# shenzebang/PDE-inverse-problem

Measured on NVIDIA B200. Metric: particle-steps/s, higher is better.
Workload: dtype bf16 GEMM operands split hi+lo (MLP weights and x; GMM centres, x and softmax weights in the integrator), f32 accumulate / epilogue / state

## Files before the change

pde_inverse_problem_b200/csrc/residual_tensor.cu:

```cuda
#include "mlp_thread.cuh"
#include "residual_common.cuh"
#include "umma.cuh"

namespace pdeip {

int mlp_residual_accumulate_fp32(int set_kind, const ResidualArgs& a, int hidden, cudaStream_t st);

namespace tc {

using namespace umma;

constexpr int H = 32;
constexpr int OP = 48;

constexpr uint32_t C_DW2 = 0, C_DW1 = 48, C_DW0 = 80, C_SLOT0 = 112, SLOT_COLS = 200;
constexpr uint32_t C_S1P1 = 0, C_S1P2 = 16;
constexpr uint32_t C_R = 32;
constexpr uint32_t C_Z0 = C_R + 0, C_Z10 = C_R + 32;
constexpr uint32_t C_Z1 = C_R + 64, C_Z11 = C_R + 96, C_Z21 = C_R + 0;
constexpr uint32_t C_U = C_R + 0, C_U1 = C_R + 48, C_U2 = C_R + 96;
constexpr uint32_t C_S0P = 176;
constexpr uint32_t C_AA2 = C_R + 0, C_AB12 = C_R + 32, C_PZ2 = C_R + 128;
constexpr uint32_t C_AA1 = C_R + 64, C_AB11 = C_R + 96, C_PZ1 = C_R + 0;
constexpr uint32_t C_G = C_R + 16;
constexpr uint32_t C_ZG0 = C_R + 64, C_ZG1 = C_R + 96, C_UG = C_R + 48;
constexpr uint32_t C_AB2 = C_R + 16, C_AA2R = C_R + 96;
constexpr uint32_t C_AB1 = C_R + 48, C_AA1R = C_R + 96;

constexpr uint32_t C_AOP = C_SLOT0 + SLOT_COLS;
constexpr uint32_t C_AOPX = C_AOP + 48;

constexpr int ZC_ZA2 = 0, ZC_ZA1 = 6, ZC_ZA0 = 10, ZC_TA = 14, ZC_TB = 20;
constexpr int AC_T = 0, AC_A1 = 4, AC_C = 8;

template <int DP, int NS>
struct Cfg {
  static constexpr int XC = DP / 8;
  static constexpr int NX = 4 * XC;
  static constexpr int KX = 2 * DP;
  static constexpr int KV = DP < 16 ? 16 : DP;
  static constexpr int XC_HI = 0, XC_LO = XC, XC_V = 2 * XC, XC_G = 3 * XC;
  static constexpr uint32_t RG_X = NX * 128, RG_A = 12 * 128, RG_Z = 24 * 128;
  static constexpr uint32_t SZ_X = 16 * RG_X, SZ_A = 16 * RG_A, SZ_Z = 16 * RG_Z;
  static constexpr uint32_t O_X = 0, O_A1 = O_X + SZ_X, O_A2 = O_A1 + SZ_A, O_Z = O_A2 + SZ_A, SLOT = O_Z + SZ_Z;
#ifndef PDEIP_TC_PIPE_X
#define PDEIP_TC_PIPE_X 1
#endif
#ifndef PDEIP_TC_STAGE
#define PDEIP_TC_STAGE 0
#endif
  static constexpr bool PIPE_X = PDEIP_TC_PIPE_X && NS == 1 && !PDEIP_TC_STAGE;
  static constexpr uint32_t O_X2 = NS * SLOT;
  static constexpr uint32_t RG_T0X = KX / 8 * 128, SZ_T0X = 4 * RG_T0X;
  static constexpr uint32_t RG_T0V = KV / 8 * 128, SZ_T0V = 4 * RG_T0V;
  static constexpr uint32_t RG_T1 = 512, SZ_T1 = 4 * RG_T1, RG_T2 = 512, SZ_T2 = 6 * RG_T2;
  static constexpr uint32_t O_T0XH = NS * SLOT + (PIPE_X ? SZ_X : 0u), O_T0XL = O_T0XH + SZ_T0X, O_T0VH = O_T0XL + SZ_T0X,
                            O_T0VL = O_T0VH + SZ_T0V, O_T1H = O_T0VL + SZ_T0V, O_T1L = O_T1H + SZ_T1,
                            O_T2H = O_T1L + SZ_T1, O_T2L = O_T2H + SZ_T2,
                            O_TGH = O_T2L + SZ_T2, O_TGL = O_TGH + (NS == 1 ? SZ_T1 : 0u),
                            O_BIAS = O_TGL + (NS == 1 ? SZ_T1 : 0u);
  static constexpr uint32_t TP_BYTES = NS == 2 ? 2048 : 4096;
#ifndef PDEIP_TC_STAGE
#define PDEIP_TC_STAGE 0
#endif
  static constexpr uint32_t STAGE_BYTES = (PDEIP_TC_STAGE && NS == 1) ? 128u * 3u * DP * 4u : 0u;
  static constexpr uint32_t O_TRUE = O_BIAS + 512, O_MISC = O_TRUE + TP_BYTES, O_STAGE = O_MISC + 128,
                            TOTAL = O_STAGE + STAGE_BYTES;
  static_assert(TOTAL <= 227u * 1024u && O_STAGE % 128 == 0 && O_X2 % 1024 == 0, "shared-memory budget");
};

#ifndef PDEIP_TC_G_CHAIN_EARLY
#define PDEIP_TC_G_CHAIN_EARLY 1
#endif
#ifndef PDEIP_TC_NLO_FWD
#define PDEIP_TC_NLO_FWD 1
#endif
#ifndef PDEIP_TC_NLO_BWD
#define PDEIP_TC_NLO_BWD 1
#endif
#ifndef PDEIP_TC_LO_FWD
#define PDEIP_TC_LO_FWD true
#endif
constexpr int kEpiThreads = 256;
constexpr int kThreads = kEpiThreads + 32;
constexpr int kLaunchThreads = 384;
#ifndef PDEIP_TC_REGS1_EPI
#define PDEIP_TC_REGS1_EPI 232
#define PDEIP_TC_REGS1_MMA 40
#endif
#ifndef PDEIP_TC_REGS2_EPI
#define PDEIP_TC_REGS2_EPI 208
#define PDEIP_TC_REGS2_MMA 88
#endif
template <int NS>
struct Regs {
  static constexpr int kEpi = NS == 2 ? PDEIP_TC_REGS2_EPI : PDEIP_TC_REGS1_EPI;
  static constexpr int kMma = NS == 2 ? PDEIP_TC_REGS2_MMA : PDEIP_TC_REGS1_MMA;
  static_assert(2 * (kEpi - 168) <= 168 - kMma && kEpi % 8 == 0 && kMma % 8 == 0 && kMma >= 24 && kEpi <= 256,
                "setmaxnreg budgets: an impossible request never returns (the kernel hangs)");
};

template <int V>
struct IC {
  static constexpr int value = V;
};

#ifdef PDEIP_TC_TRACE
constexpr int kTraceTiles = 64;
#define TC_TRACE(k) do { if (trace_on) atomicAdd(reinterpret_cast<unsigned long long*>(trace) + (ph * 2 + s) * 8 + (k), (unsigned long long)clock64()); } while (0)
#define TC_FINE(k) do { if (trace_on && ph == 4) atomicAdd(reinterpret_cast<unsigned long long*>(trace) + 240 + s * 8 + (k), (unsigned long long)clock64()); } while (0)
#define TC_TRACE_DECL_MMA                                                     \
  long long* trace = reinterpret_cast<long long*>(status) + 512;              \
  const bool trace_on = blockIdx.x == 0 && base >= tile_begin + (int64_t)16 * tile_stride && base < tile_begin + (int64_t)(16 + kTraceTiles) * tile_stride
#else
#define TC_TRACE(k) do { } while (0)
#define TC_FINE(k) do { } while (0)
#define TC_TRACE_DECL_MMA do { } while (0)
#endif

#ifdef PDEIP_TC_PROBE
#define TC_PROBE(id, unit0, arr, n)                                                              \
  do {                                                                                           \
    if (probe_on) {                                                                              \
      for (int _i = 0; _i < (n); ++_i) probe[((id) * 128 + row) * 48 + (unit0) + _i] = (arr)[_i]; \
    }                                                                                            \
  } while (0)
#else
#define TC_PROBE(id, unit0, arr, n) do { } while (0)
#endif

template <bool PROXY_FENCE = true>
__device__ __forceinline__ void epi_arrive(int slot) {
  if constexpr (PROXY_FENCE) fence_async_smem();
  fence_before_sync();
  asm volatile("bar.arrive %0, %1;" ::"r"(1 + slot), "n"(kThreads) : "memory");
}
__device__ __forceinline__ void mma_wait_operands(int slot) {
  asm volatile("bar.sync %0, %1;" ::"r"(1 + slot), "n"(kThreads) : "memory");
  fence_after_sync();
}

struct Desc {
  uint32_t lo, hi;
};
__device__ __forceinline__ Desc mk_desc(uint32_t saddr, uint32_t lbo_bytes, uint32_t sbo_bytes) {
  Desc d;
  d.lo = ((saddr >> 4) & 0x3FFFu) | (((lbo_bytes >> 4) & 0x3FFFu) << 16);
  d.hi = ((sbo_bytes >> 4) & 0x3FFFu) | (1u << 14);
  return d;
}
__device__ __forceinline__ Desc mk_desc16(uint32_t base16, uint32_t off_bytes, uint32_t lbo_bytes, uint32_t sbo_bytes) {
  Desc d;
  d.lo = base16 + ((off_bytes >> 4) | (((lbo_bytes >> 4) & 0x3FFFu) << 16));
  d.hi = ((sbo_bytes >> 4) & 0x3FFFu) | (1u << 14);
  return d;
}
__device__ __forceinline__ uint32_t opaque(uint32_t v) {
  uint32_t r;
  asm volatile("mov.u32 %0, %1;" : "=r"(r) : "r"(v));
  return r;
}
__device__ __forceinline__ void mma(uint32_t d_tmem, Desc a, uint32_t a_adv, Desc b, uint32_t b_adv, uint32_t idesc,
                                    uint32_t accumulate) {
  asm volatile(
      "{\n\t"
      ".reg .pred p;\n\t"
      ".reg .b64 da, db;\n\t"
      "mov.b64 da, {%1, %2};\n\t"
      "mov.b64 db, {%3, %4};\n\t"
      "setp.ne.b32 p, %6, 0;\n\t"
      "tcgen05.mma.cta_group::1.kind::f16 [%0], da, db, %5, p;\n\t"
      "}\n" ::"r"(d_tmem),
      "r"(a.lo + (a_adv >> 4)), "r"(a.hi), "r"(b.lo + (b_adv >> 4)), "r"(b.hi), "r"(idesc), "r"(accumulate)
      : "memory");
}

__device__ __forceinline__ void mma_ts(uint32_t d_tmem, uint32_t a_tmem, Desc b, uint32_t b_adv, uint32_t idesc,
                                       uint32_t accumulate) {
  asm volatile(
      "{\n\t"
      ".reg .pred p;\n\t"
      ".reg .b64 db;\n\t"
      "mov.b64 db, {%2, %3};\n\t"
      "setp.ne.b32 p, %5, 0;\n\t"
      "tcgen05.mma.cta_group::1.kind::f16 [%0], [%1], db, %4, p;\n\t"
      "}\n" ::"r"(d_tmem),
      "r"(a_tmem), "r"(b.lo + (b_adv >> 4)), "r"(b.hi), "r"(idesc), "r"(accumulate)
      : "memory");
}
template <int K, int N, int NG, bool LO = true, int NLO = NG>
__device__ __forceinline__ void mm_fwd_ts(const uint32_t (&d)[NG], const uint32_t (&a_col)[NG], Desc w_hi, Desc w_lo) {
  constexpr uint32_t idesc = make_idesc(N, 0, 0);
#pragma unroll
  for (int k = 0; k < K; k += 16)
#pragma unroll
    for (int g = 0; g < NG; ++g) mma_ts(d[g], a_col[g] + (k >> 1), w_hi, k * 16, idesc, k > 0 ? 1u : 0u);
  if constexpr (LO) {
#pragma unroll
    for (int k = 0; k < K; k += 16)
#pragma unroll
      for (int g = 0; g < NLO; ++g) mma_ts(d[g], a_col[g] + (k >> 1), w_lo, k * 16, idesc, 1u);
  }
}
template <int K, int N, int NG, bool LO = true, int NLO = NG>
__device__ __forceinline__ void mm_bwd_ts(const uint32_t (&d)[NG], const uint32_t (&a_col)[NG], Desc w_hi_m, Desc w_lo_m,
                                          uint32_t w_rg) {
  constexpr uint32_t idesc = make_idesc(N, 0, 1);
#pragma unroll
  for (int k = 0; k < K; k += 16)
#pragma unroll
    for (int g = 0; g < NG; ++g) mma_ts(d[g], a_col[g] + (k >> 1), w_hi_m, (k >> 3) * w_rg, idesc, k > 0 ? 1u : 0u);
  if constexpr (LO) {
#pragma unroll
    for (int k = 0; k < K; k += 16)
#pragma unroll
      for (int g = 0; g < NLO; ++g) mma_ts(d[g], a_col[g] + (k >> 1), w_lo_m, (k >> 3) * w_rg, idesc, 1u);
  }
}

template <int K, int N, int NG, bool LO = true, int NLO = NG>
__device__ __forceinline__ void mm_fwd(const uint32_t (&d)[NG], Desc a, const uint32_t (&a_off)[NG], Desc w_hi, Desc w_lo) {
  constexpr uint32_t idesc = make_idesc(N, 0, 0);
#pragma unroll
  for (int k = 0; k < K; k += 16)
#pragma unroll
    for (int g = 0; g < NG; ++g) mma(d[g], a, a_off[g] + k * 16, w_hi, k * 16, idesc, k > 0 ? 1u : 0u);
  if constexpr (LO) {
#pragma unroll
    for (int k = 0; k < K; k += 16)
#pragma unroll
      for (int g = 0; g < NLO; ++g) mma(d[g], a, a_off[g] + k * 16, w_lo, k * 16, idesc, 1u);
  }
}
template <int K, int N, int NG, bool LO = true, int NLO = NG>
__device__ __forceinline__ void mm_bwd(const uint32_t (&d)[NG], Desc a, const uint32_t (&a_off)[NG], Desc w_hi_m,
                                       Desc w_lo_m, uint32_t w_rg) {
  constexpr uint32_t idesc = make_idesc(N, 0, 1);
#pragma unroll
  for (int k = 0; k < K; k += 16)
#pragma unroll
    for (int g = 0; g < NG; ++g) mma(d[g], a, a_off[g] + k * 16, w_hi_m, (k >> 3) * w_rg, idesc, k > 0 ? 1u : 0u);
  if constexpr (LO) {
#pragma unroll
    for (int k = 0; k < K; k += 16)
#pragma unroll
      for (int g = 0; g < NLO; ++g) mma(d[g], a, a_off[g] + k * 16, w_lo_m, (k >> 3) * w_rg, idesc, 1u);
  }
}
template <int N>
__device__ __forceinline__ void mm_outer(uint32_t d, Desc a_m, uint32_t a_off, uint32_t a_rg, Desc b_m, uint32_t b_off,
                                         uint32_t b_rg, uint32_t accumulate) {
  constexpr uint32_t idesc = (make_idesc(N, 1, 1) & ~(0x1Fu << 24)) | ((uint32_t)(64 >> 4) << 24);
#pragma unroll
  for (int k = 0; k < 128; k += 16)
    mma(d, a_m, a_off + (k >> 3) * a_rg, b_m, b_off + (k >> 3) * b_rg, idesc, k > 0 ? 1u : accumulate);
}

__device__ __forceinline__ float tanh_fast(float x) {
  float y;
  asm("tanh.approx.f32 %0, %1;" : "=f"(y) : "f"(x));
  return y;
}

__device__ __forceinline__ uint32_t pack2(float a, float b) {
  __nv_bfloat162 p = __floats2bfloat162_rn(a, b);
  return *reinterpret_cast<uint32_t*>(&p);
}
__device__ __forceinline__ float bf_lo(uint32_t w) { return __uint_as_float(w << 16); }
__device__ __forceinline__ float bf_hi(uint32_t w) { return __uint_as_float(w & 0xffff0000u); }
__device__ __forceinline__ void load_chunk(const uint8_t* tile, uint32_t off, float* v) {
  const uint4 q = *reinterpret_cast<const uint4*>(tile + off);
  v[0] = bf_lo(q.x); v[1] = bf_hi(q.x); v[2] = bf_lo(q.y); v[3] = bf_hi(q.y);
  v[4] = bf_lo(q.z); v[5] = bf_hi(q.z); v[6] = bf_lo(q.w); v[7] = bf_hi(q.w);
}
__device__ __forceinline__ void put_chunk(uint8_t* tile, uint32_t off, const float* v) {
  uint4 q;
  q.x = pack2(v[0], v[1]); q.y = pack2(v[2], v[3]); q.z = pack2(v[4], v[5]); q.w = pack2(v[6], v[7]);
  *reinterpret_cast<uint4*>(tile + off) = q;
}
__device__ __forceinline__ void mbar_expect_tx(uint32_t mbar, uint32_t bytes) {
  asm volatile("mbarrier.arrive.expect_tx.shared::cta.b64 _, [%0], %1;" ::"r"(mbar), "r"(bytes) : "memory");
}
__device__ __forceinline__ void bulk_g2s(uint32_t dst_smem, const void* src, uint32_t bytes, uint32_t mbar) {
  asm volatile("cp.async.bulk.shared::cluster.global.mbarrier::complete_tx::bytes [%0], [%1], %2, [%3];" ::"r"(dst_smem),
               "l"(src), "r"(bytes), "r"(mbar)
               : "memory");
}
__device__ __forceinline__ void tm_st4(uint32_t taddr, const uint32_t* r);
template <bool TS>
__device__ __forceinline__ void put_op(uint8_t* tile, uint32_t off, uint32_t taddr, const float* v) {
  uint4 q;
  q.x = pack2(v[0], v[1]); q.y = pack2(v[2], v[3]); q.z = pack2(v[4], v[5]); q.w = pack2(v[6], v[7]);
  *reinterpret_cast<uint4*>(tile + off) = q;
  if constexpr (TS) tm_st4(taddr, reinterpret_cast<const uint32_t*>(&q));
}
__device__ __forceinline__ void tm_ld8(uint32_t taddr, uint32_t* r) {
  asm volatile("tcgen05.ld.sync.aligned.32x32b.x8.b32 {%0,%1,%2,%3,%4,%5,%6,%7}, [%8];"
               : "=r"(r[0]), "=r"(r[1]), "=r"(r[2]), "=r"(r[3]), "=r"(r[4]), "=r"(r[5]), "=r"(r[6]), "=r"(r[7])
               : "r"(taddr)
               : "memory");
}
__device__ __forceinline__ void tm_ld4(uint32_t taddr, uint32_t* r) {
  asm volatile("tcgen05.ld.sync.aligned.32x32b.x4.b32 {%0,%1,%2,%3}, [%4];"
               : "=r"(r[0]), "=r"(r[1]), "=r"(r[2]), "=r"(r[3])
               : "r"(taddr)
               : "memory");
}
__device__ __forceinline__ void tm_ld16(uint32_t taddr, uint32_t* r) {
  asm volatile(
      "tcgen05.ld.sync.aligned.32x32b.x16.b32 {%0,%1,%2,%3,%4,%5,%6,%7,%8,%9,%10,%11,%12,%13,%14,%15}, [%16];"
      : "=r"(r[0]), "=r"(r[1]), "=r"(r[2]), "=r"(r[3]), "=r"(r[4]), "=r"(r[5]), "=r"(r[6]), "=r"(r[7]), "=r"(r[8]),
        "=r"(r[9]), "=r"(r[10]), "=r"(r[11]), "=r"(r[12]), "=r"(r[13]), "=r"(r[14]), "=r"(r[15])
      : "r"(taddr)
      : "memory");
}
__device__ __forceinline__ void tm_wait_ld() { asm volatile("tcgen05.wait::ld.sync.aligned;" ::: "memory"); }
__device__ __forceinline__ void tm_wait_st() { asm volatile("tcgen05.wait::st.sync.aligned;" ::: "memory"); }
__device__ __forceinline__ void tm_st8(uint32_t taddr, const uint32_t* r) {
  asm volatile("tcgen05.st.sync.aligned.32x32b.x8.b32 [%0], {%1,%2,%3,%4,%5,%6,%7,%8};" ::"r"(taddr), "r"(r[0]),
               "r"(r[1]), "r"(r[2]), "r"(r[3]), "r"(r[4]), "r"(r[5]), "r"(r[6]), "r"(r[7])
               : "memory");
}
__device__ __forceinline__ void tm_st4(uint32_t taddr, const uint32_t* r) {
  asm volatile("tcgen05.st.sync.aligned.32x32b.x4.b32 [%0], {%1,%2,%3,%4};" ::"r"(taddr), "r"(r[0]), "r"(r[1]),
               "r"(r[2]), "r"(r[3])
               : "memory");
}
template <int NU>
__device__ __forceinline__ void tm_ldf(uint32_t taddr, float* v) {
  uint32_t* r = reinterpret_cast<uint32_t*>(v);
  tm_ld16(taddr, r);
  if constexpr (NU == 24) tm_ld8(taddr + 16, r + 16);
}
template <int NU>
__device__ __forceinline__ void tm_ldp(uint32_t taddr, uint32_t* r) {
  tm_ld8(taddr, r);
  if constexpr (NU == 24) tm_ld4(taddr + 8, r + 8);
}
template <int NU>
__device__ __forceinline__ void tm_park(uint32_t taddr, const float* v) {
  uint32_t r[NU / 2];
#pragma unroll
  for (int i = 0; i < NU / 2; ++i) r[i] = pack2(v[2 * i], v[2 * i + 1]);
  if constexpr (NU == 8) {
    tm_st4(taddr, r);
  } else {
    tm_st8(taddr, r);
    if constexpr (NU == 24) tm_st4(taddr + 8, r + 8);
  }
  tm_wait_st();
}

template <int DP>
__device__ __noinline__ void true_grad_chunk(const ResidualArgs& a, const float* __restrict__ tp, int64_t p, int dimw,
                                             int cg, float* gt) {
  const int d = a.d;
  float x[DP];
#pragma unroll
  for (int u = 0; u < DP; ++u)
    x[u] = (p >= 0 && u < d) ? __ldg(a.points + elem_index(a.layout, p, u, a.n_points, dimw)) : 0.f;
  if (a.tg.kind == PDEIP_DRIFT_LINEAR) {
#pragma unroll
    for (int e = 0; e < 8; ++e) {
      const int u = cg * 8 + e;
      float acc = 0.f;
      if (u < d) {
#pragma unroll
        for (int k = 0; k < DP; ++k)
          if (k < d) acc = fmaf(tp[u * d + k], x[k], acc);
      }
      gt[e] = acc;
    }
  } else {
    float m = -INFINITY;
    for (int k = 0; k < a.tg.n_gaussian; ++k) {
      float s2 = 0.f;
#pragma unroll
      for (int u = 0; u < DP; ++u)
        if (u < d) {
          const float r = x[u] - tp[k * d + u];
          s2 = fmaf(r, r, s2);
        }
      m = fmaxf(m, -0.5f * a.tg.inv_sigma2 * s2);
    }
    float se = 0.f, wm[8];
#pragma unroll
    for (int e = 0; e < 8; ++e) wm[e] = 0.f;
    for (int k = 0; k < a.tg.n_gaussian; ++k) {
      float s2 = 0.f;
#pragma unroll
      for (int u = 0; u < DP; ++u)
        if (u < d) {
          const float r = x[u] - tp[k * d + u];
          s2 = fmaf(r, r, s2);
        }
      const float ek = __expf(-0.5f * a.tg.inv_sigma2 * s2 - m);
      se += ek;
#pragma unroll
      for (int e = 0; e < 8; ++e)
        if (cg * 8 + e < d) wm[e] = fmaf(ek, tp[k * d + cg * 8 + e], wm[e]);
    }
    const float inv = 1.f / se;
#pragma unroll
    for (int e = 0; e < 8; ++e) gt[e] = (cg * 8 + e < d) ? (x[cg * 8 + e] - wm[e] * inv) * a.tg.inv_sigma2 : 0.f;
  }
}
__device__ __forceinline__ float unp(const uint32_t* r, int i) { return (i & 1) ? bf_hi(r[i >> 1]) : bf_lo(r[i >> 1]); }

#ifndef PDEIP_TC_PACKED
#define PDEIP_TC_PACKED 1
#endif
__device__ __forceinline__ float2 pr(const float* v, int i) { return make_float2(v[2 * i], v[2 * i + 1]); }
__device__ __forceinline__ void st2(float* v, int i, float2 x) { v[2 * i] = x.x; v[2 * i + 1] = x.y; }
__device__ __forceinline__ float2 unp2(const uint32_t* r, int i) { return make_float2(bf_lo(r[i]), bf_hi(r[i])); }
__device__ __forceinline__ float2 bc2(float x) { return make_float2(x, x); }

constexpr int kModeKfp0T = 0, kModeBnd = 1, kModeFp0T = 2;
template <int DP, int NS, int MODE>
__global__ void __launch_bounds__(kLaunchThreads, 1) mlp_residual_tc_kernel(const ResidualArgs a, int* status) {
  constexpr bool BND = MODE == kModeBnd, FPM = MODE == kModeFp0T;
#ifndef PDEIP_TC_TS
#define PDEIP_TC_TS 1
#endif
  constexpr bool kTS = PDEIP_TC_TS && NS == 1;
#ifndef PDEIP_TC_GRAM
#define PDEIP_TC_GRAM 1
#endif
  constexpr bool kGram = PDEIP_TC_GRAM && NS == 1;
#ifndef PDEIP_TC_TWO_STAGE
#define PDEIP_TC_TWO_STAGE 1
#endif
  constexpr bool kTwoStage = PDEIP_TC_TWO_STAGE && kTS;
  constexpr bool kPipeX = Cfg<DP, NS>::PIPE_X;
  constexpr bool kPipeFlow = kPipeX;
  using S = Cfg<DP, NS>;
  extern __shared__ __align__(1024) uint8_t sm[];
  const int tid = threadIdx.x, warp = tid >> 5, lane = tid & 31;
  const bool is_mma_warp = warp == kEpiThreads / 32;
  const int q = warp & 3;
  const int half = (warp >> 2) & 1;
  const int row = q * 32 + lane;
  const int d = a.d;
  const MlpShape<H> sh{d, 2};
  const int P = sh.num_params();
  float* bias_s = reinterpret_cast<float*>(sm + S::O_BIAS);
  float* tp = reinterpret_cast<float*>(sm + S::O_TRUE);
  uint64_t* mbar_p = reinterpret_cast<uint64_t*>(sm + S::O_MISC);
  uint32_t* tmem_p = reinterpret_cast<uint32_t*>(sm + S::O_MISC + 64);

  const uint32_t fpd = FPM ? (uint32_t)a.fp_dirs : 1u;
  const int64_t n_tiles_all = (a.n_points + 127) / 128 * fpd;
  const int64_t per_cta = ((n_tiles_all + gridDim.x - 1) / gridDim.x + NS - 1) / NS * NS;
  const int64_t tile_begin = (int64_t)blockIdx.x * per_cta;
  if (tile_begin >= n_tiles_all) return;
  const int64_t n_tiles = tile_begin + per_cta < n_tiles_all ? tile_begin + per_cta : n_tiles_all;

  if (warp == 0) {
    tmem_alloc(smem_u32(tmem_p), 512);
    tmem_relinquish();
  }
  if (tid == 0) {
    for (int s = 0; s < NS; ++s) mbar_init(smem_u32(mbar_p + s), 1);
    mbar_init(smem_u32(mbar_p + 4), 1);
    fence_mbar_init();
  }
  for (uint32_t o = tid * 16; o < S::O_BIAS; o += kLaunchThreads * 16) *reinterpret_cast<uint4*>(sm + o) = make_uint4(0, 0, 0, 0);
  if constexpr (S::PIPE_X)
    for (uint32_t o = tid * 16; o < S::SZ_X; o += kLaunchThreads * 16) *reinterpret_cast<uint4*>(sm + S::O_X2 + o) = make_uint4(0, 0, 0, 0);
  __syncthreads();
  {
    const float* W0 = a.params + sh.w_off(0);
    const float* W1 = a.params + sh.w_off(1);
    const float* W2 = a.params + sh.w_off(2);
    auto put = [&](uint32_t o_hi, uint32_t o_lo, uint32_t rg, int r, int c, float w) {
      const __nv_bfloat16 hi = __float2bfloat16_rn(w);
      const __nv_bfloat16 lo = __float2bfloat16_rn(w - __bfloat162float(hi));
      const uint32_t off = chunk_off(r, c >> 3, rg) + (uint32_t)(c & 7) * 2u;
      *reinterpret_cast<__nv_bfloat16*>(sm + o_hi + off) = hi;
      *reinterpret_cast<__nv_bfloat16*>(sm + o_lo + off) = lo;
    };
    for (int idx = tid; idx < 32 * S::KX; idx += kLaunchThreads) {
      const int r = idx / S::KX, c = idx % S::KX, ci = c % DP;
      put(S::O_T0XH, S::O_T0XL, S::RG_T0X, r, c, ci < d ? W0[ci * H + r] : 0.f);
    }
    for (int idx = tid; idx < 32 * S::KV; idx += kLaunchThreads) {
      const int r = idx / S::KV, c = idx % S::KV;
      put(S::O_T0VH, S::O_T0VL, S::RG_T0V, r, c, c < d ? W0[c * H + r] : 0.f);
    }
    for (int idx = tid; idx < 32 * 32; idx += kLaunchThreads) {
      const int r = idx / 32, c = idx % 32;
      put(S::O_T1H, S::O_T1L, S::RG_T1, r, c, W1[c * H + r]);
    }
    for (int idx = tid; idx < OP * 32; idx += kLaunchThreads) {
      const int r = idx / 32, c = idx % 32;
      put(S::O_T2H, S::O_T2L, S::RG_T2, r, c, r < kOut ? W2[c * kOut + r] : 0.f);
    }
    if constexpr (kGram) {
      const float sc = 0.125f / (float)fpd;
      for (int idx = tid; idx < 32 * 32; idx += kLaunchThreads) {
        const int r = idx / 32, c = idx % 32;
        float acc = 0.f;
        for (int k = 0; k < d; ++k) acc = fmaf(W0[k * H + r], W0[k * H + c], acc);
        put(S::O_TGH, S::O_TGL, S::RG_T1, r, c, sc * acc);
      }
    }
    for (int j = tid; j < 32; j += kLaunchThreads) {
      bias_s[j] = a.params[sh.b_off(0) + j];
      bias_s[32 + j] = a.params[sh.b_off(1) + j];
    }
    for (int j = tid; j < OP; j += kLaunchThreads) bias_s[64 + j] = j < kOut ? a.params[sh.b_off(2) + j] : 0.f;
    int ntg = 0;
    if (a.tg.kind == PDEIP_DRIFT_LINEAR) ntg = d * d;
    else if (a.tg.kind == PDEIP_DRIFT_GMM) ntg = a.tg.n_gaussian * d;
    for (int i = tid; i < ntg; i += kLaunchThreads) tp[i] = a.tg.params[i];
  }
  fence_async_smem();
  fence_before_sync();
  __syncthreads();
  fence_after_sync();

  const uint32_t TB = *tmem_p;
  const int64_t tile_stride = NS;

  if (warp >= kEpiThreads / 32) {
    asm volatile("setmaxnreg.dec.sync.aligned.u32 %0;" ::"n"(Regs<NS>::kMma));
  }
  if (is_mma_warp) {
    const uint32_t sm16 = smem_u32(sm) >> 4;
    constexpr uint32_t CH = 128;
    uint32_t dw_started = 0;
    constexpr bool kCChainsEarly = PDEIP_TC_G_CHAIN_EARLY && NS == 2;
    constexpr int kNloFwd = BND ? 2 : PDEIP_TC_NLO_FWD;
    constexpr int kNloBwd = BND ? 2 : PDEIP_TC_NLO_BWD;
    uint32_t xb = 0;
    uint32_t tsb = 0;
#pragma unroll 1
    for (int64_t base = tile_begin; base < n_tiles; base += tile_stride) {
#pragma unroll 1
      for (int ph = (kPipeFlow && base != tile_begin) ? 1 : 0; ph < 12; ++ph) {
        if (kGram && ph == 6) continue;
#pragma unroll 1
        for (int s = 0; s < NS; ++s) {
          const uint32_t w16 = opaque(sm16), b16 = opaque(sm16 + (uint32_t)s * (S::SLOT >> 4));
          const uint32_t x16 = kPipeX ? opaque(sm16 + (xb ? (S::O_X2 >> 4) : 0u)) : b16;
          const uint32_t x16n = kPipeX ? opaque(sm16 + (xb ? 0u : (S::O_X2 >> 4))) : b16;
          const uint32_t TBo = opaque(TB);
          const uint32_t TS = TBo + C_SLOT0 + (uint32_t)s * SLOT_COLS;
          const uint32_t mb = smem_u32(mbar_p + s);
          const uint32_t AOP = TBo + C_AOP;
          const Desc T0XHK = mk_desc16(w16, S::O_T0XH, 128, S::RG_T0X), T0XLK = mk_desc16(w16, S::O_T0XL, 128, S::RG_T0X);
          const Desc T0VHK = mk_desc16(w16, S::O_T0VH, 128, S::RG_T0V), T0VLK = mk_desc16(w16, S::O_T0VL, 128, S::RG_T0V);
          const Desc T1HK = mk_desc16(w16, S::O_T1H, 128, S::RG_T1), T1LK = mk_desc16(w16, S::O_T1L, 128, S::RG_T1);
          const Desc T2HK = mk_desc16(w16, S::O_T2H, 128, S::RG_T2), T2LK = mk_desc16(w16, S::O_T2L, 128, S::RG_T2);
          const Desc TGHK = mk_desc16(w16, S::O_TGH, 128, S::RG_T1), TGLK = mk_desc16(w16, S::O_TGL, 128, S::RG_T1);
          const Desc T0VHM = mk_desc16(w16, S::O_T0VH, S::RG_T0V, 128), T0VLM = mk_desc16(w16, S::O_T0VL, S::RG_T0V, 128);
          const Desc T1HM = mk_desc16(w16, S::O_T1H, S::RG_T1, 128), T1LM = mk_desc16(w16, S::O_T1L, S::RG_T1, 128);
          const Desc T2HM = mk_desc16(w16, S::O_T2H, S::RG_T2, 128), T2LM = mk_desc16(w16, S::O_T2L, S::RG_T2, 128);
          const Desc XK = mk_desc16(x16, S::O_X, 128, S::RG_X), A1K = mk_desc16(b16, S::O_A1, 128, S::RG_A),
                     A2K = mk_desc16(b16, S::O_A2, 128, S::RG_A), ZK = mk_desc16(b16, S::O_Z, 128, S::RG_Z);
          const Desc XM = mk_desc16(x16, S::O_X, S::RG_X, 128), ZM = mk_desc16(b16, S::O_Z, S::RG_Z, 128);
          const uint32_t AOPX = kPipeX ? TBo + C_AOPX : AOP;
          auto issue_p0 = [&](const Desc xk) {
            if constexpr (kTS) {
              mm_fwd_ts<S::KX, 32, 1>({TS + C_Z0}, {AOPX}, T0XHK, T0XLK);
              mm_fwd_ts<S::KV, 32, 1, (PDEIP_TC_NLO_FWD >= 2 || BND)>({TS + C_Z10}, {AOPX + S::KX / 2}, T0VHK, T0VLK);
            } else {
              mm_fwd<S::KX, 32, 1>({TS + C_Z0}, xk, {S::XC_HI * CH}, T0XHK, T0XLK);
              mm_fwd<S::KV, 32, 1, (PDEIP_TC_NLO_FWD >= 2 || BND)>({TS + C_Z10}, xk, {S::XC_V * CH}, T0VHK, T0VLK);
            }
          };
          TC_TRACE_DECL_MMA;
          mma_wait_operands(s);
          if (elect_one()) {
            TC_TRACE(4);
            switch (ph) {
              case 0: {
                issue_p0(XK);
                commit(mb);
              } break;
              case 1: {
                if constexpr (kTS) mm_fwd_ts<32, 32, 3, PDEIP_TC_LO_FWD, kNloFwd>({TS + C_Z1, TS + C_Z11, TS + C_Z21}, {AOP + 4 * AC_T, AOP + 4 * AC_A1, AOP + 4 * AC_C}, T1HK, T1LK);
                else mm_fwd<32, 32, 3, PDEIP_TC_LO_FWD, kNloFwd>({TS + C_Z1, TS + C_Z11, TS + C_Z21}, A1K, {AC_T * CH, AC_A1 * CH, AC_C * CH}, T1HK, T1LK);
                commit(mb);
              } break;
              case 2: {
                if constexpr (kTS) mm_fwd_ts<32, OP, 3, PDEIP_TC_LO_FWD, kNloFwd>({TS + C_U, TS + C_U1, TS + C_U2}, {AOP + 4 * AC_T, AOP + 4 * AC_A1, AOP + 4 * AC_C}, T2HK, T2LK);
                else mm_fwd<32, OP, 3, PDEIP_TC_LO_FWD, kNloFwd>({TS + C_U, TS + C_U1, TS + C_U2}, A2K, {AC_T * CH, AC_A1 * CH, AC_C * CH}, T2HK, T2LK);
                commit(mb);
              } break;
              case 3: {
                if constexpr (kTS) mm_bwd_ts<OP, 32, 2, true, kNloBwd>({TS + C_AA2, TS + C_AB12}, {AOP, AOP + 24}, T2HM, T2LM, S::RG_T2);
                else mm_bwd<OP, 32, 2, true, kNloBwd>({TS + C_AA2, TS + C_AB12}, ZK, {ZC_ZA2 * CH, ZC_TA * CH}, T2HM, T2LM, S::RG_T2);
                commit(mb);
              } break;
              case 4: {
                if constexpr (kTS) mm_bwd_ts<32, 32, 2, true, kNloBwd>({TS + C_AA1, TS + C_AB11}, {AOP, AOP + 16}, T1HM, T1LM, S::RG_T1);
                else mm_bwd<32, 32, 2, true, kNloBwd>({TS + C_AA1, TS + C_AB11}, ZK, {ZC_ZA1 * CH, ZC_TB * CH}, T1HM, T1LM, S::RG_T1);
                commit(mb);
              } break;
              case 5: {
                if constexpr (kTS) mm_bwd_ts<32, S::KV, 1>({TS + C_G}, {AOP}, T0VHM, T0VLM, S::RG_T0V);
                else mm_bwd<32, S::KV, 1>({TS + C_G}, ZK, {ZC_ZA0 * CH}, T0VHM, T0VLM, S::RG_T0V);
                if constexpr (kGram) {
                  if constexpr (kTS) mm_fwd_ts<32, 32, 1, true>({TS + C_ZG0}, {AOP}, TGHK, TGLK);
                  else mm_fwd<32, 32, 1, true>({TS + C_ZG0}, ZK, {ZC_ZA0 * CH}, TGHK, TGLK);
                }
                commit(mb);
              } break;
              case 6: {
                if constexpr (kTS) mm_fwd_ts<S::KV, 32, 1, false>({TS + C_ZG0}, {AOP}, T0VHK, T0VLK);
                else mm_fwd<S::KV, 32, 1, false>({TS + C_ZG0}, XK, {S::XC_G * CH}, T0VHK, T0VLK);
                commit(mb);
#if PDEIP_TC_G_CHAIN_EARLY
                mm_outer<32>(TBo + C_DW0, XM, S::XC_G * CH, S::RG_X, ZM, ZC_ZA0 * CH, S::RG_Z, 1u);
#endif
              } break;
              case 7: {
                if constexpr (kTS) mm_fwd_ts<32, 32, 1, false>({TS + C_ZG1}, {AOP}, T1HK, T1LK);
                else mm_fwd<32, 32, 1, false>({TS + C_ZG1}, A1K, {AC_A1 * CH}, T1HK, T1LK);
                commit(mb);
                if constexpr (kGram && !kTwoStage)
                  mm_outer<32>(TBo + C_DW0, XM, S::XC_G * CH, S::RG_X, ZM, ZC_ZA0 * CH, S::RG_Z, 1u);
                if constexpr (kCChainsEarly) {
                  const Desc A1M = mk_desc16(b16, S::O_A1, S::RG_A, 128);
                  mm_outer<32>(TBo + C_DW1, A1M, AC_C * CH, S::RG_A, ZM, ZC_ZA1 * CH, S::RG_Z, 1u);
                }
              } break;
              case 8: {
                if constexpr (kTS) mm_fwd_ts<32, OP, 1, false>({TS + C_UG}, {AOP}, T2HK, T2LK);
                else mm_fwd<32, OP, 1, false>({TS + C_UG}, A2K, {AC_A1 * CH}, T2HK, T2LK);
                commit(mb);
                if constexpr (kCChainsEarly) {
                  const Desc A2M = mk_desc16(b16, S::O_A2, S::RG_A, 128);
                  mm_outer<OP>(TBo + C_DW2, A2M, AC_C * CH, S::RG_A, ZM, ZC_ZA2 * CH, S::RG_Z, 1u);
                }
              } break;
              case 9: {
                if constexpr (kTS) {
                  mm_bwd_ts<OP, 32, 1, BND, 1>({TS + C_AB2}, {AOP}, T2HM, T2LM, S::RG_T2);
                  mm_bwd<OP, 32, 1, false>({TS + C_AA2R}, ZK, {ZC_ZA2 * CH}, T2HM, T2LM, S::RG_T2);
                } else {
                  mm_bwd<OP, 32, 2, BND, 1>({TS + C_AB2, TS + C_AA2R}, ZK, {ZC_TA * CH, ZC_ZA2 * CH}, T2HM, T2LM, S::RG_T2);
                }
                commit(mb);
              } break;
              case 10: {
                if constexpr (kTS) {
                  mm_bwd_ts<32, 32, 1, BND, 1>({TS + C_AB1}, {AOP}, T1HM, T1LM, S::RG_T1);
                  mm_bwd<32, 32, 1, false>({TS + C_AA1R}, ZK, {ZC_ZA1 * CH}, T1HM, T1LM, S::RG_T1);
                } else {
                  mm_bwd<32, 32, 2, BND, 1>({TS + C_AB1, TS + C_AA1R}, ZK, {ZC_TB * CH, ZC_ZA1 * CH}, T1HM, T1LM, S::RG_T1);
                }
                commit(mb);
              } break;
              default: {
                const bool p0_next = kPipeFlow && base + tile_stride < n_tiles;
                if (p0_next) {
                  issue_p0(mk_desc16(x16n, S::O_X, 128, S::RG_X));
                  commit(mb);
                }
                if constexpr (!kTwoStage) {
                  mm_outer<32>(TBo + C_DW0, XM, S::XC_HI * CH, S::RG_X, ZM, ZC_TA * CH, S::RG_Z, 1u);
#ifdef PDEIP_TC_XLO_DW
                  mm_outer<32>(TBo + C_DW0, XM, S::XC_LO * CH, S::RG_X, ZM, ZC_TA * CH, S::RG_Z, 1u);
#endif
#if !PDEIP_TC_G_CHAIN_EARLY
                  mm_outer<32>(TBo + C_DW0, XM, S::XC_G * CH, S::RG_X, ZM, ZC_ZA0 * CH, S::RG_Z, 1u);
#endif
                  if (!p0_next) commit(mb);
                }
              } break;
            }
            TC_TRACE(6);
          }
          __syncwarp();
        }
        if (ph == 3 || ph == 4 || ph == 5 || ph == 9 || ph == 10 || (kTwoStage && (ph == 7 || ph == 11))) {
#pragma unroll 1
          for (int s = 0; s < NS; ++s) {
            if constexpr (kTwoStage) {
              asm volatile("bar.sync %0, %1;" ::"r"(4 + (int)tsb), "n"(kThreads) : "memory");
              tsb ^= 1u;
              fence_after_sync();
            }
            const uint32_t b16 = opaque(sm16 + (uint32_t)s * (S::SLOT >> 4)), TBo = opaque(TB);
            const uint32_t x16 = kPipeX ? opaque(sm16 + (xb ? (S::O_X2 >> 4) : 0u)) : b16;
            const Desc XM = mk_desc16(x16, S::O_X, S::RG_X, 128), A1M = mk_desc16(b16, S::O_A1, S::RG_A, 128),
                       A2M = mk_desc16(b16, S::O_A2, S::RG_A, 128), ZM = mk_desc16(b16, S::O_Z, S::RG_Z, 128);
            const uint32_t acc_first = (dw_started | (uint32_t)s) ? 1u : 0u;
            if (elect_one()) {
              switch (ph) {
                case 3:
                  mm_outer<OP>(TBo + C_DW2, A2M, AC_A1 * CH, S::RG_A, ZM, ZC_TA * CH, S::RG_Z, acc_first);
                  break;
                case 4:
                  mm_outer<32>(TBo + C_DW1, A1M, AC_A1 * CH, S::RG_A, ZM, ZC_TB * CH, S::RG_Z, acc_first);
                  break;
                case 5:
                  mm_outer<32>(TBo + C_DW0, XM, S::XC_V * CH, S::RG_X, ZM, ZC_TA * CH, S::RG_Z, acc_first);
                  break;
                case 9:
                  mm_outer<OP>(TBo + C_DW2, A2M, AC_T * CH, S::RG_A, ZM, ZC_TA * CH, S::RG_Z, 1u);
                  if constexpr (!kCChainsEarly)
                    mm_outer<OP>(TBo + C_DW2, A2M, AC_C * CH, S::RG_A, ZM, ZC_ZA2 * CH, S::RG_Z, 1u);
                  break;
                case 10:
                  mm_outer<32>(TBo + C_DW1, A1M, AC_T * CH, S::RG_A, ZM, ZC_TB * CH, S::RG_Z, 1u);
                  if constexpr (!kCChainsEarly)
                    mm_outer<32>(TBo + C_DW1, A1M, AC_C * CH, S::RG_A, ZM, ZC_ZA1 * CH, S::RG_Z, 1u);
                  break;
                case 7:
                  if constexpr (kGram) mm_outer<32>(TBo + C_DW0, XM, S::XC_G * CH, S::RG_X, ZM, ZC_ZA0 * CH, S::RG_Z, 1u);
                  break;
                default: {
                  mm_outer<32>(TBo + C_DW0, XM, S::XC_HI * CH, S::RG_X, ZM, ZC_TA * CH, S::RG_Z, 1u);
#ifdef PDEIP_TC_XLO_DW
                  mm_outer<32>(TBo + C_DW0, XM, S::XC_LO * CH, S::RG_X, ZM, ZC_TA * CH, S::RG_Z, 1u);
#endif
#if !PDEIP_TC_G_CHAIN_EARLY
                  mm_outer<32>(TBo + C_DW0, XM, S::XC_G * CH, S::RG_X, ZM, ZC_ZA0 * CH, S::RG_Z, 1u);
#endif
                  if (!(kPipeFlow && base + tile_stride < n_tiles)) commit(smem_u32(mbar_p + s));
                } break;
              }
            }
            __syncwarp();
          }
        }
      }
      dw_started = 1u;
      xb ^= 1u;
    }
  } else if (warp < kEpiThreads / 32) {
    asm volatile("setmaxnreg.inc.sync.aligned.u32 %0;" ::"n"(Regs<NS>::kEpi));
    bool ok = true;
    uint32_t par = 0;
#ifdef PDEIP_TC_PROBE
    float* probe = reinterpret_cast<float*>(status) + 2048;
#endif
    float db0[16], db1[16], db2[24];
#pragma unroll
    for (int i = 0; i < 16; ++i) { db0[i] = 0.f; db1[i] = 0.f; }
#pragma unroll
    for (int i = 0; i < 24; ++i) db2[i] = 0.f;
    float sum_g2 = 0.f, sum_gt2 = 0.f, sum_gd2 = 0.f, sum_d1 = 0.f, sum_d2 = 0.f;
    const float gamma = a.coef, gamma4 = 4.f * a.coef;
    const float cgw = 1.f / (float)fpd;
    const int dimw = (FPM ? d : 2 * d) + (a.tg.kind == PDEIP_DRIFT_IN_POINTS ? d : 0);
    const uint32_t offX = (uint32_t)(row & 7) * 16u + (uint32_t)(row >> 3) * S::RG_X;
    const uint32_t offA = (uint32_t)(row & 7) * 16u + (uint32_t)(row >> 3) * S::RG_A;
    const uint32_t offZ = (uint32_t)(row & 7) * 16u + (uint32_t)(row >> 3) * S::RG_Z;
    const uint32_t LA0 = TB + ((uint32_t)(q * 32) << 16) + C_SLOT0;
    const uint32_t LOP = TB + ((uint32_t)(q * 32) << 16) + C_AOP;
    const int u16 = 16 * half, u24 = 24 * half;
    constexpr int NI = (3 * S::XC + 1) / 2;
    float xin0[NI][8], xin1[NI][8];
    const bool fast_in = !FPM && a.layout == PDEIP_LAYOUT_BLOCK128 && d == DP;
    auto load_into = [&](float (&xin)[NI][8], int64_t t, const int i0 = 0, const int i1 = 64) {
      if (fast_in) {
        const int64_t pp = t * 128 + row;
        const bool inside = t < n_tiles && pp < a.n_points;
        const float* const pb = a.points + (inside ? t * (int64_t)(128 * dimw) + row : (int64_t)0) + half * (8 * 128);
        const bool has_gt = a.tg.kind == PDEIP_DRIFT_IN_POINTS;
#pragma unroll
        for (int i = 0; i < NI; ++i) {
          if (i < i0 || i >= i1) continue;
          if (half + 2 * i >= 3 * S::XC) continue;
          if (half + 2 * i >= 2 * S::XC && !has_gt) continue;
#pragma unroll
          for (int e = 0; e < 8; ++e) xin[i][e] = __ldg(pb + (16 * i + e) * 128);
        }
        return;
      }
      const int64_t cstride = comp_stride(a.layout, a.n_points);
      const uint32_t tq = FPM ? (uint32_t)t / fpd : 0u;
      const int dir = FPM ? (int)((uint32_t)t - tq * fpd) : -1;
      const int64_t pp = (FPM ? (int64_t)tq : t) * 128 + row;
      const int64_t pc = (t < n_tiles && pp < a.n_points) ? pp : 0;
      const float* const pbase = a.points + point_base(a.layout, pc, dimw);
#pragma unroll
      for (int i = 0; i < NI; ++i) {
        if (i < i0 || i >= i1) continue;
        const int j = half + 2 * i;
        const int band = (j / S::XC) < 3 ? (j / S::XC) : 0, cg = j % S::XC;
        const int bandc = (band < 2 || a.tg.kind == PDEIP_DRIFT_IN_POINTS) ? band : 0;
        const int bandm = FPM ? (bandc == 2 ? 1 : 0) : bandc;
#pragma unroll
        for (int e = 0; e < 8; ++e) {
          const int u = cg * 8 + e;
          const int uc = u < d ? u : 0;
          const float val = __ldg(pbase + (bandm * d + uc) * cstride);
          xin[i][e] = (FPM && band == 1) ? (u == dir ? 1.f : 0.f) : val;
        }
      }
    };
    constexpr bool kStage = PDEIP_TC_STAGE && NS == 1;
    const bool use_stage = kStage && a.layout == PDEIP_LAYOUT_BLOCK128 && (reinterpret_cast<uintptr_t>(a.points) & 15u) == 0;
    const float* const stage = reinterpret_cast<const float*>(sm + S::O_STAGE) + row;
    const uint32_t stage_mbar = smem_u32(mbar_p + 4);
    uint32_t spar = 0;
    auto stage_issue = [&](int64_t t) {
      if (t >= n_tiles) return;
      const int64_t pt = FPM ? (int64_t)((uint32_t)t / fpd) : t;
      const uint32_t bytes = 512u * (uint32_t)dimw;
      mbar_expect_tx(stage_mbar, bytes);
      bulk_g2s(smem_u32(sm + S::O_STAGE), a.points + pt * 128 * dimw, bytes, stage_mbar);
    };
    if (use_stage && tid == 0) stage_issue(tile_begin);
    auto load_inputs = [&](int s, int64_t t, const int i0 = 0, const int i1 = 64) {
      if (NS == 2 && s == 1) load_into(xin1, t, i0, i1);
      else load_into(xin0, t, i0, i1);
    };
#ifndef PDEIP_TC_L2_PREFETCH
#define PDEIP_TC_L2_PREFETCH 1
#endif
    auto prefetch_inputs = [&](int64_t t) {
      if (FPM || t >= n_tiles || (t + 1) * 128 > a.n_points) return;
      if (a.layout == PDEIP_LAYOUT_SOA) {
        if ((a.n_points & 3) == 0 && half == 0 && row < dimw)
          asm volatile("cp.async.bulk.prefetch.L2.global [%0], %1;" ::"l"(a.points + (int64_t)row * a.n_points + t * 128),
                       "r"(512u)
                       : "memory");
      } else if (half == 0 && row == 0) {
        asm volatile("cp.async.bulk.prefetch.L2.global [%0], %1;" ::"l"(a.points + t * 128 * dimw),
                     "r"((uint32_t)(512 * dimw))
                     : "memory");
      }
    };
#if !PDEIP_TC_L2_PREFETCH
    load_inputs(0, tile_begin);
    if constexpr (NS == 2) load_inputs(1, tile_begin + 1);
#endif

    bool first = true;
    int64_t base = tile_begin;
    uint32_t xb = 0;
    uint32_t tsb = 0;
    const uint32_t LOPX = kPipeX ? TB + ((uint32_t)(q * 32) << 16) + C_AOPX : LOP;
    auto emit_x = [&](const float (&xin)[NI][8], const bool valid_t, uint8_t* const Xd) {
#pragma unroll
      for (int i = 0; i < NI; ++i) {
        const int j = half + 2 * i;
        const int band = j / S::XC, cg = j % S::XC;
        if (band == 0) {
          float hi[8], lo[8];
#pragma unroll
          for (int e = 0; e < 8; ++e) {
            const float xv = (valid_t && cg * 8 + e < d) ? xin[i][e] : 0.f;
            hi[e] = __bfloat162float(__float2bfloat16_rn(xv));
            lo[e] = xv - hi[e];
          }
          put_op<kTS>(Xd, (S::XC_HI + cg) * 128, LOPX + 4 * cg, hi);
          put_op<kTS>(Xd, (S::XC_LO + cg) * 128, LOPX + 4 * (S::XC + cg), lo);
        } else if (band == 1) {
          float vv[8];
#pragma unroll
          for (int e = 0; e < 8; ++e) vv[e] = (valid_t && cg * 8 + e < d) ? xin[i][e] : 0.f;
          put_op<kTS>(Xd, (S::XC_V + cg) * 128, LOPX + S::KX / 2 + 4 * cg, vv);
        }
      }
    };

    auto phase = [&](auto PHc, const int s) {
      constexpr int ph = decltype(PHc)::value;
      uint8_t* const X = sm + (kPipeX ? (xb ? S::O_X2 : 0u) : (uint32_t)s * S::SLOT) + S::O_X + offX;
      uint8_t* const A1 = sm + (uint32_t)s * S::SLOT + S::O_A1 + offA;
      uint8_t* const A2 = sm + (uint32_t)s * S::SLOT + S::O_A2 + offA;
      uint8_t* const Z = sm + (uint32_t)s * S::SLOT + S::O_Z + offZ;
      const uint32_t LA = LA0 + (uint32_t)s * SLOT_COLS;
      const int64_t tile = base + s;
      const int64_t p = (FPM ? (int64_t)((uint32_t)tile / fpd) : tile) * 128 + row;
      const bool valid = tile < n_tiles && p < a.n_points;
      const float mk = valid ? 1.f : 0.f;
#ifdef PDEIP_TC_PROBE
      const bool probe_on = blockIdx.x == 0 && tile == 0;
#endif
#ifdef PDEIP_TC_TRACE
      long long* trace = reinterpret_cast<long long*>(status) + 512;
      const bool trace_on = blockIdx.x == 0 && tid == 0 && base >= tile_begin + (int64_t)16 * tile_stride &&
                            base < tile_begin + (int64_t)(16 + kTraceTiles) * tile_stride;
#endif
      auto wait_gemm = [&]() {
        TC_TRACE(0);
        if (!(ph == 0 && first)) {
          if (ok && !mbar_wait(smem_u32(mbar_p + s), (par >> s) & 1u)) {
            ok = false;
            atomicExch(status, 1);
          }
          par ^= 1u << s;
          TC_TRACE(3);
          fence_after_sync();
        }
        TC_TRACE(1);
      };
      constexpr bool kEarlyLoads = true;
#if PDEIP_TC_L2_PREFETCH
      if constexpr (ph == 0) {
        if (!use_stage) load_inputs(s, tile);
      }
#endif
      if constexpr (kStage && ph == 0) {
        if (use_stage) {
          if (ok && !mbar_wait(stage_mbar, spar)) {
            ok = false;
            atomicExch(status, 1);
          }
          spar ^= 1u;
          const int dir = FPM ? (int)((uint32_t)tile % fpd) : -1;
#pragma unroll
          for (int i = 0; i < NI; ++i) {
            const int j = half + 2 * i;
            const int band = (j / S::XC) < 3 ? (j / S::XC) : 0, cg = j % S::XC;
            if (band < 2) {
#pragma unroll
              for (int e = 0; e < 8; ++e) {
                const int u = cg * 8 + e;
                const float val = stage[(band * d + (u < d ? u : 0)) * 128];
                xin0[i][e] = (FPM && band == 1) ? (u == dir ? 1.f : 0.f) : val;
              }
            }
          }
        }
      }
      if constexpr (ph <= 3 || ph == 6 || !kEarlyLoads) wait_gemm();
      if constexpr (ph == 0) {
        if (NS == 2 && s == 1) emit_x(xin1, valid, X);
        else emit_x(xin0, valid, X);
      } else if constexpr (ph == 1 || ph == 2) {
        constexpr bool l1 = ph == 1;
        uint8_t* const At = l1 ? A1 : A2;
        float z0[16], z1[16], z2[16];
        tm_ldf<16>(LA + (l1 ? C_Z0 : C_Z1) + u16, z0);
        tm_ldf<16>(LA + (l1 ? C_Z10 : C_Z11) + u16, z1);
        if constexpr (!l1) tm_ldf<16>(LA + C_Z21 + u16, z2);
        float bb[16];
#pragma unroll
        for (int i = 0; i < 4; ++i)
          *reinterpret_cast<float4*>(bb + 4 * i) = *reinterpret_cast<const float4*>(bias_s + (l1 ? 0 : 32) + u16 + 4 * i);
        tm_wait_ld();
        float t[16], s1[16], q1[16], q2[16];
#if PDEIP_TC_PACKED
#pragma unroll
        for (int i = 0; i < 8; ++i) {
          const float2 zb = __fadd2_rn(pr(z0, i), pr(bb, i));
          const float2 t2 = make_float2(tanh_fast(zb.x), tanh_fast(zb.y));
          const float2 s2 = __ffma2_rn(__fmul2_rn(t2, bc2(-1.f)), t2, bc2(1.f));
          const float2 z12 = pr(z1, i);
          const float2 q = __fmul2_rn(s2, z12);
          float2 r = __fmul2_rn(__fmul2_rn(t2, q), z12);
          if constexpr (!l1) r = __ffma2_rn(s2, pr(z2, i), r);
          st2(t, i, t2); st2(s1, i, s2); st2(q1, i, q); st2(q2, i, r);
        }
#else
#pragma unroll
        for (int i = 0; i < 16; ++i) {
          t[i] = tanh_fast(z0[i] + bb[i]);
          s1[i] = fmaf(-t[i], t[i], 1.f);
          q1[i] = s1[i] * z1[i];
          const float w = t[i] * q1[i];
          q2[i] = l1 ? w * z1[i] : fmaf(s1[i], z2[i], w * z1[i]);
        }
#endif
#pragma unroll
        for (int c = 0; c < 2; ++c) {
          put_op<kTS>(At, (AC_T + 2 * half + c) * 128, LOP + 4 * (AC_T + 2 * half + c), t + 8 * c);
          put_op<kTS>(At, (AC_A1 + 2 * half + c) * 128, LOP + 4 * (AC_A1 + 2 * half + c), q1 + 8 * c);
          put_op<kTS>(At, (AC_C + 2 * half + c) * 128, LOP + 4 * (AC_C + 2 * half + c), q2 + 8 * c);
        }
        tm_park<16>(LA + (l1 ? C_S1P1 : C_S1P2) + 8 * half, s1);
        TC_PROBE(l1 ? 0 : 3, u16, t, 16);
        TC_PROBE(l1 ? 1 : 4, u16, q1, 16);
        TC_PROBE(l1 ? 2 : 5, u16, q2, 16);
      } else if constexpr (ph == 3) {
        float u[24], u1[24], u2[24];
        tm_ldf<24>(LA + C_U + u24, u);
        tm_ldf<24>(LA + C_U1 + u24, u1);
        tm_ldf<24>(LA + C_U2 + u24, u2);
        float bb[24];
#pragma unroll
        for (int i = 0; i < 6; ++i)
          *reinterpret_cast<float4*>(bb + 4 * i) = *reinterpret_cast<const float4*>(bias_s + 64 + u24 + 4 * i);
        tm_wait_ld();
        const float k8 = BND ? 0.f : 8.f * mk, kg = (BND ? 2.f * a.coef : gamma4) * mk;
        float d1 = 0.f, d2a = 0.f, d2b = 0.f;
        float za[24], sv[24], sp[24];
#if PDEIP_TC_PACKED
        {
          float2 e1 = bc2(0.f), e2a = bc2(0.f), e2b = bc2(0.f);
          const float2 k82 = bc2(k8), nk82 = bc2(-k8), kg2 = bc2(kg);
#pragma unroll
          for (int i = 0; i < 12; ++i) {
            const float2 uu = __fadd2_rn(pr(u, i), pr(bb, i));
            const float2 v1 = pr(u1, i), v2 = pr(u2, i);
            e1 = __ffma2_rn(uu, v1, e1);
            e2a = __ffma2_rn(v1, v1, e2a);
            e2b = __ffma2_rn(uu, v2, e2b);
            st2(za, i, __fmul2_rn(k82, uu));
            st2(sv, i, __ffma2_rn(nk82, v1, __fmul2_rn(kg2, uu)));
            st2(sp, i, __ffma2_rn(k82, v2, __fmul2_rn(kg2, v1)));
          }
          d1 = e1.x + e1.y; d2a = e2a.x + e2a.y; d2b = e2b.x + e2b.y;
        }
#else
#pragma unroll
        for (int i = 0; i < 24; ++i) {
          const float uu = u[i] + bb[i];
          d1 = fmaf(uu, u1[i], d1);
          d2a = fmaf(u1[i], u1[i], d2a);
          d2b = fmaf(uu, u2[i], d2b);
          za[i] = k8 * uu;
          sv[i] = fmaf(-k8, u1[i], kg * uu);
          sp[i] = fmaf(k8, u2[i], kg * u1[i]);
        }
#endif
#pragma unroll
        for (int c = 0; c < 3; ++c) {
          put_op<kTS>(Z, (ZC_ZA2 + 3 * half + c) * 128, LOP + 4 * (3 * half + c), za + 8 * c);
          put_op<kTS>(Z, (ZC_TA + 3 * half + c) * 128, LOP + 24 + 4 * (3 * half + c), sv + 8 * c);
        }
        tm_park<24>(LA + C_S0P + 12 * half, sp);
        sum_d1 = fmaf(2.f * mk, d1, sum_d1);
        sum_d2 = fmaf(mk, 2.f * d2a - 4.f * d2b, sum_d2);
        TC_PROBE(6, u24, za, 24);
        TC_PROBE(7, u24, sv, 24);
        TC_PROBE(8, u24, sp, 24);
      } else if constexpr (ph == 4 || ph == 5) {
        if constexpr (kPipeFlow && ph == 4) prefetch_inputs(tile + tile_stride);
        constexpr bool l2 = ph == 4;
        const uint8_t* At = l2 ? A2 : A1;
        float aa[16], ab1[16], t[16], a1[16];
        uint32_t s1p[8];
        tm_ldp<16>(LA + (l2 ? C_S1P2 : C_S1P1) + 8 * half, s1p);
#pragma unroll
        for (int c = 0; c < 2; ++c) {
          load_chunk(At, (AC_T + 2 * half + c) * 128, t + 8 * c);
          load_chunk(At, (AC_A1 + 2 * half + c) * 128, a1 + 8 * c);
        }
        tm_wait_ld();
        if constexpr (kEarlyLoads) wait_gemm();
        tm_ldf<16>(LA + (l2 ? C_AA2 : C_AA1) + u16, aa);
        tm_ldf<16>(LA + (l2 ? C_AB12 : C_AB11) + u16, ab1);
        tm_wait_ld();
        TC_FINE(0);
        float za[16], zb[16], pz[16];
#if PDEIP_TC_PACKED
#pragma unroll
        for (int i = 0; i < 8; ++i) {
          const float2 s2 = unp2(s1p, i), aa2 = pr(aa, i), a12 = pr(a1, i), ab2 = pr(ab1, i);
          const float2 tt = __fmul2_rn(pr(t, i), bc2(2.f));
          const float2 qq = __fmul2_rn(aa2, a12);
          st2(za, i, __fmul2_rn(aa2, s2));
          st2(zb, i, __ffma2_rn(tt, qq, __fmul2_rn(s2, ab2)));
          st2(pz, i, __fmul2_rn(a12, __ffma2_rn(__fmul2_rn(tt, bc2(-1.f)), ab2, qq)));
        }
#else
#pragma unroll
        for (int i = 0; i < 16; ++i) {
          const float s1 = unp(s1p, i);
          za[i] = aa[i] * s1;
          const float qq = aa[i] * a1[i];
          zb[i] = fmaf(2.f * t[i], qq, s1 * ab1[i]);
          pz[i] = a1[i] * fmaf(-2.f * t[i], ab1[i], qq);
        }
#endif
#pragma unroll
        for (int c = 0; c < 2; ++c) {
          put_op<kTS>(Z, ((l2 ? ZC_ZA1 : ZC_ZA0) + 2 * half + c) * 128, LOP + 4 * (2 * half + c), za + 8 * c);
          put_op<(kTS && l2)>(Z, ((l2 ? ZC_TB : ZC_TA) + 2 * half + c) * 128, LOP + 16 + 4 * (2 * half + c), zb + 8 * c);
        }
        TC_FINE(1);
        tm_park<16>(LA + (l2 ? C_PZ2 : C_PZ1) + 8 * half, pz);
        TC_FINE(2);
        TC_PROBE(l2 ? 9 : 12, u16, za, 16);
        TC_PROBE(l2 ? 10 : 13, u16, zb, 16);
        TC_PROBE(l2 ? 11 : 14, u16, pz, 16);
      } else if constexpr (ph == 6) {
#pragma unroll
        for (int i = 0; i < NI; ++i) {
          const int j = half + 2 * i;
          const int band = j / S::XC, cg = j % S::XC;
          const bool own_sum = a.tg.kind == PDEIP_DRIFT_IN_POINTS ? band == 2 : band == 0;
          if (j < 3 * S::XC && (band == 0 || own_sum)) {
            float g4[8], gv[8], gt[8];
            tm_ld8(LA + C_G + 8 * cg, reinterpret_cast<uint32_t*>(g4));
            tm_wait_ld();
#pragma unroll
            for (int e = 0; e < 8; ++e) {
              gv[e] = 0.25f * g4[e];
              gt[e] = 0.f;
            }
            if (band == 0) {
              float gh[8];
#pragma unroll
              for (int e = 0; e < 8; ++e) gh[e] = (0.125f * cgw) * g4[e];
              put_op<kTS>(X, (S::XC_G + cg) * 128, LOP + 4 * cg, gh);
              TC_PROBE(15, cg * 8, gv, 8);
            }
            if (own_sum) {
              const float mkc = mk * cgw;
              if (a.tg.kind == PDEIP_DRIFT_IN_POINTS) {
#pragma unroll
                for (int e = 0; e < 8; ++e) {
                  const int u = cg * 8 + e;
                  float val;
                  if (kStage && use_stage) val = stage[((FPM ? d : 2 * d) + (u < d ? u : 0)) * 128];
                  else val = (NS == 2 && s == 1) ? xin1[i][e] : xin0[i][e];
                  gt[e] = (valid && u < d) ? val : 0.f;
                }
              } else if (a.tg.kind == PDEIP_DRIFT_LINEAR || a.tg.kind == PDEIP_DRIFT_GMM) {
                true_grad_chunk<DP>(a, tp, valid ? p : (int64_t)-1, dimw, cg, gt);
              }
#pragma unroll
              for (int e = 0; e < 8; ++e) {
                const float df = gt[e] - gv[e];
                sum_g2 = fmaf(mkc * gv[e], gv[e], sum_g2);
                sum_gt2 = fmaf(mkc * gt[e], gt[e], sum_gt2);
                sum_gd2 = fmaf(mkc * df, df, sum_gd2);
              }
            }
          }
        }
      } else if constexpr (ph == 7 || ph == 8) {
        constexpr bool l1 = ph == 7;
        uint8_t* const At = l1 ? A1 : A2;
        float zg[16], a2[16];
        uint32_t s1p[8];
        tm_ldp<16>(LA + (l1 ? C_S1P1 : C_S1P2) + 8 * half, s1p);
#pragma unroll
        for (int c = 0; c < 2; ++c) load_chunk(At, (AC_C + 2 * half + c) * 128, a2 + 8 * c);
        tm_wait_ld();
        if constexpr (kEarlyLoads && !(kGram && l1)) wait_gemm();
        if constexpr (kStage && l1) {
          if (use_stage && tid == 0) stage_issue(tile + tile_stride);
        }
        tm_ldf<16>(LA + (l1 ? C_ZG0 : C_ZG1) + u16, zg);
        tm_wait_ld();
        float ag[16], cc[16];
#if PDEIP_TC_PACKED
#pragma unroll
        for (int i = 0; i < 8; ++i) {
          const float2 g2 = __fmul2_rn(unp2(s1p, i), pr(zg, i));
          st2(ag, i, g2);
          st2(cc, i, __fadd2_rn(pr(a2, i), g2));
        }
#else
#pragma unroll
        for (int i = 0; i < 16; ++i) {
          ag[i] = unp(s1p, i) * zg[i];
          cc[i] = a2[i] + ag[i];
        }
#endif
#pragma unroll
        for (int c = 0; c < 2; ++c) {
          put_op<kTS>(At, (AC_A1 + 2 * half + c) * 128, LOP + 4 * (2 * half + c), ag + 8 * c);
          put_chunk(At, (AC_C + 2 * half + c) * 128, cc + 8 * c);
        }
        TC_PROBE(l1 ? 16 : 17, u16, cc, 16);
      } else if constexpr (ph == 9) {
        float ug[24], s0[24];
        uint32_t spp[12];
        tm_ldp<24>(LA + C_S0P + 12 * half, spp);
        tm_wait_ld();
        if constexpr (kEarlyLoads) wait_gemm();
        tm_ldf<24>(LA + C_UG + u24, ug);
        tm_wait_ld();
#if PDEIP_TC_PACKED
#pragma unroll
        for (int i = 0; i < 12; ++i) {
          const float2 v = __ffma2_rn(bc2(8.f), pr(ug, i), unp2(spp, i));
          st2(s0, i, v);
          st2(db2, i, __fadd2_rn(pr(db2, i), v));
        }
#else
#pragma unroll
        for (int i = 0; i < 24; ++i) {
          s0[i] = fmaf(8.f, ug[i], unp(spp, i));
          db2[i] += s0[i];
        }
#endif
#pragma unroll
        for (int c = 0; c < 3; ++c) put_op<kTS>(Z, (ZC_TA + 3 * half + c) * 128, LOP + 4 * (3 * half + c), s0 + 8 * c);
        TC_PROBE(18, u24, s0, 24);
      } else {
        constexpr bool l2 = ph == 10;
#if PDEIP_TC_L2_PREFETCH
        if constexpr (l2) {
          if constexpr (kPipeFlow) {
            if (tile + tile_stride < n_tiles) load_inputs(s, tile + tile_stride, 0, 2);
          } else if (!use_stage) {
            prefetch_inputs(tile + tile_stride);
          }
        }
#else
        if constexpr (l2) load_inputs(s, tile + tile_stride);
#endif
        const uint8_t* At = l2 ? A2 : A1;
        float ab[16], aa[16], t[16], cc[16];
        uint32_t s1p[8], pzp[8];
        tm_ldp<16>(LA + (l2 ? C_S1P2 : C_S1P1) + 8 * half, s1p);
        tm_ldp<16>(LA + (l2 ? C_PZ2 : C_PZ1) + 8 * half, pzp);
#pragma unroll
        for (int c = 0; c < 2; ++c) {
          load_chunk(At, (AC_T + 2 * half + c) * 128, t + 8 * c);
          load_chunk(At, (AC_C + 2 * half + c) * 128, cc + 8 * c);
        }
        tm_wait_ld();
        if constexpr (kEarlyLoads) wait_gemm();
        tm_ldf<16>(LA + (l2 ? C_AB2 : C_AB1) + u16, ab);
        tm_ldf<16>(LA + (l2 ? C_AA2R : C_AA1R) + u16, aa);
        tm_wait_ld();
        float zb[16];
#if PDEIP_TC_PACKED
#pragma unroll
        for (int i = 0; i < 8; ++i) {
          const float2 m0 = __ffma2_rn(unp2(s1p, i), pr(ab, i), unp2(pzp, i));
          const float2 ta = __fmul2_rn(__fmul2_rn(pr(t, i), bc2(-2.f)), pr(aa, i));
          const float2 v = __ffma2_rn(ta, pr(cc, i), m0);
          st2(zb, i, v);
          if (l2) st2(db1, i, __fadd2_rn(pr(db1, i), v));
          else st2(db0, i, __fadd2_rn(pr(db0, i), v));
        }
#else
#pragma unroll
        for (int i = 0; i < 16; ++i) {
          const float m0 = fmaf(unp(s1p, i), ab[i], unp(pzp, i));
          zb[i] = fmaf(-2.f * t[i] * aa[i], cc[i], m0);
          if (l2) db1[i] += zb[i];
          else db0[i] += zb[i];
        }
#endif
#pragma unroll
        for (int c = 0; c < 2; ++c)
          put_op<(kTS && l2)>(Z, ((l2 ? ZC_TB : ZC_TA) + 2 * half + c) * 128, LOP + 4 * (2 * half + c), zb + 8 * c);
        TC_PROBE(l2 ? 19 : 20, u16, zb, 16);
      }
      if constexpr (!(kGram && ph == 6)) {
        if constexpr (kTS) tm_wait_st();
        TC_TRACE(7);
        if constexpr (kTwoStage && (ph == 3 || ph == 4 || ph == 5 || ph == 7 || ph == 9 || ph == 10 || ph == 11)) {
          epi_arrive<false>(s);
          fence_async_smem();
          asm volatile("bar.arrive %0, %1;" ::"r"(4 + (int)tsb), "n"(kThreads) : "memory");
          tsb ^= 1u;
        } else {
#ifdef PDEIP_TC_TRACE
        fence_async_smem();
        TC_FINE(3);
        fence_before_sync();
        TC_FINE(4);
        asm volatile("bar.arrive %0, %1;" ::"r"(1 + s), "n"(kThreads) : "memory");
#else
        constexpr bool kNeedProxyFence = !(kTS && (ph == 0 || ph == 1 || ph == 2 || ph == 8));
        epi_arrive<kNeedProxyFence>(s);
#endif
        }
        TC_TRACE(2);
      }
      if constexpr (kPipeFlow && ph == 10) {
        const int64_t tn = tile + tile_stride;
        const int64_t pn = (FPM ? (int64_t)((uint32_t)tn / fpd) : tn) * 128 + row;
        if (tn < n_tiles) {
          load_inputs(s, tn, 2, 64);
          emit_x(xin0, pn < a.n_points, sm + (xb ? 0u : S::O_X2) + S::O_X + offX);
        }
      }
    };
#define PDEIP_TC_PHASE(PH)                       \
  _Pragma("unroll 1") for (int s_ = 0; s_ < NS; ++s_) phase(IC<PH>{}, s_);

#pragma unroll 1
    for (; base < n_tiles; base += tile_stride) {
      if (!kPipeFlow || first) { PDEIP_TC_PHASE(0) }
      PDEIP_TC_PHASE(1) PDEIP_TC_PHASE(2) PDEIP_TC_PHASE(3) PDEIP_TC_PHASE(4) PDEIP_TC_PHASE(5)
      PDEIP_TC_PHASE(6) PDEIP_TC_PHASE(7) PDEIP_TC_PHASE(8) PDEIP_TC_PHASE(9) PDEIP_TC_PHASE(10) PDEIP_TC_PHASE(11)
      first = false;
      xb ^= 1u;
    }
#undef PDEIP_TC_PHASE
#pragma unroll
    for (int s = 0; s < NS; ++s) {
      if (ok && !mbar_wait(smem_u32(mbar_p + s), (par >> s) & 1u)) {
        ok = false;
        atomicExch(status, 1);
      }
    }
    fence_after_sync();
    asm volatile("bar.sync 3, %0;" ::"n"(kEpiThreads) : "memory");

    float* part = a.ws + (int64_t)blockIdx.x * a.pstride;
    float* red = reinterpret_cast<float*>(sm);
    const float wt = a.weight;
    if (ok && q < 2) {
      const uint32_t LQ = TB + ((uint32_t)(q * 32) << 16);
      const int iu = 16 * q + lane;
      float w2[24], w1[16], w0[16];
      tm_ldf<24>(LQ + C_DW2 + u24, w2);
      tm_ldf<16>(LQ + C_DW1 + u16, w1);
      tm_ldf<16>(LQ + C_DW0 + u16, w0);
      tm_wait_ld();
      if (lane < 16) {
#pragma unroll
        for (int i = 0; i < 24; ++i)
          if (u24 + i < kOut) part[sh.w_off(2) + iu * kOut + u24 + i] += wt * w2[i];
#pragma unroll
        for (int i = 0; i < 16; ++i) part[sh.w_off(1) + iu * H + u16 + i] += wt * w1[i];
        if (iu < d) {
#pragma unroll
          for (int i = 0; i < 16; ++i) part[sh.w_off(0) + iu * H + u16 + i] += wt * w0[i];
        }
      }
    }
#pragma unroll
    for (int i = 0; i < 16; ++i) {
      const float r0 = warp_sum(db0[i]), r1 = warp_sum(db1[i]);
      if (lane == 0) {
        red[q * 128 + u16 + i] = r0;
        red[q * 128 + 32 + u16 + i] = r1;
      }
    }
#pragma unroll
    for (int i = 0; i < 24; ++i) {
      const float r2 = warp_sum(db2[i]);
      if (lane == 0) red[q * 128 + 64 + u24 + i] = r2;
    }
    {
      const float sums5[5] = {sum_g2, sum_gt2, sum_gd2, sum_d1, sum_d2};
#pragma unroll
      for (int k = 0; k < 5; ++k) {
        const float sk = warp_sum(sums5[k]);
        if (lane == 0) red[512 + warp * 8 + k] = sk;
      }
    }
    asm volatile("bar.sync 3, %0;" ::"n"(kEpiThreads) : "memory");
    if (ok) {
      if (tid < 112) {
        const float v = (red[tid] + red[128 + tid]) + (red[256 + tid] + red[384 + tid]);
        if (tid < 32) part[sh.b_off(0) + tid] += wt * v;
        else if (tid < 64) part[sh.b_off(1) + tid - 32] += wt * v;
        else if (tid - 64 < kOut) part[sh.b_off(2) + tid - 64] += wt * v;
      }
      if (tid == 128) {
        float t5[5] = {0.f, 0.f, 0.f, 0.f, 0.f};
        for (int w = 0; w < kEpiThreads / 32; ++w)
          for (int k = 0; k < 5; ++k) t5[k] += red[512 + w * 8 + k];
        const float g2 = wt * t5[0], gt2 = wt * t5[1], gd2 = wt * t5[2], D1 = wt * t5[3], D2 = wt * t5[4];
        if constexpr (BND) {
          part[P + PDEIP_SUM_BOUNDARY] += a.coef * D1;
          part[P + PDEIP_SUM_LOSS] += a.coef * D1;
        } else {
          part[P + PDEIP_SUM_G2] += g2;
          part[P + PDEIP_SUM_GTRUE2] += gt2;
          part[P + PDEIP_SUM_GT] += gd2;
          if (!FPM) part[P + PDEIP_SUM_D1] += D1;
          part[P + PDEIP_SUM_D2] += D2;
          part[P + PDEIP_SUM_LOSS] += g2 + gt2 - 2.f * D2 + 2.f * gamma * D1;
        }
      }
    }
  }
  fence_before_sync();
  __syncthreads();
  if (warp == 0) tmem_dealloc(TB, 512);
}

}

int* tensor_status_word() {
  static int* w[64] = {nullptr};
  int dev = 0;
  if (cudaGetDevice(&dev) != cudaSuccess || dev < 0 || dev >= 64) return nullptr;
  if (!w[dev]) {
    const size_t bytes = 8192 + 24 * 128 * 48 * sizeof(float);
    if (cudaMalloc(&w[dev], bytes) != cudaSuccess) return nullptr;
    cudaMemset(w[dev], 0, bytes);
  }
  return w[dev];
}

#ifdef PDEIP_HAVE_TENSOR_PATH
template <int DP, int NS, int MODE>
static int launch_tc(const ResidualArgs& a, int* status, cudaStream_t st) {
  using S = tc::Cfg<DP, NS>;
  auto kern = tc::mlp_residual_tc_kernel<DP, NS, MODE>;
  PDEIP_REQUIRE(true_grad_floats(a.tg, a.d) * sizeof(float) <= S::TP_BYTES, PDEIP_ERR_UNSUPPORTED,
                "tensor path: true-gradient parameters exceed %u bytes", (unsigned)S::TP_BYTES);
  PDEIP_CUDA_OK(cudaFuncSetAttribute(kern, cudaFuncAttributeMaxDynamicSharedMemorySize, (int)S::TOTAL));
  kern<<<residual_grid(), tc::kLaunchThreads, S::TOTAL, st>>>(a, status);
  PDEIP_LAUNCH_OK();
  return PDEIP_OK;
}

int mlp_residual_accumulate_tensor(int set_kind, const ResidualArgs& a, int hidden, cudaStream_t st) {
  if (set_kind != PDEIP_SET_KFP_0T && set_kind != PDEIP_SET_FP_0T && set_kind != PDEIP_SET_KFP_BOUNDARY)
    return mlp_residual_accumulate_fp32(set_kind, a, hidden, st);
  PDEIP_REQUIRE(hidden == 32 && a.layers == 2, PDEIP_ERR_UNSUPPORTED,
                "tensor path is built for hidden_dim == 32, layers == 2 (got %d, %d)", hidden, a.layers);
  PDEIP_REQUIRE(a.d >= 1 && a.d <= 32, PDEIP_ERR_UNSUPPORTED, "tensor path supports 1 <= d <= 32 (got %d)", a.d);
  int* status = tensor_status_word();
  PDEIP_REQUIRE(status != nullptr, PDEIP_ERR_CUDA, "cannot allocate the tensor-path status word");
  ResidualArgs b = a;
  int mode = tc::kModeKfp0T;
  if (set_kind == PDEIP_SET_FP_0T) {
    PDEIP_REQUIRE((a.n_points + 127) / 128 * (int64_t)a.d < ((int64_t)1 << 31), PDEIP_ERR_UNSUPPORTED,
                  "FP tensor path: n_points * d / 128 must stay below 2^31");
    b.fp_dirs = a.d;
    b.coef = 0.f;
    mode = tc::kModeFp0T;
  } else if (set_kind == PDEIP_SET_KFP_BOUNDARY) {
    b.tg.kind = PDEIP_DRIFT_NONE;
    mode = tc::kModeBnd;
  }
#define PDEIP_TC_DISPATCH(DP, NS)                                                     \
  (mode == tc::kModeKfp0T ? launch_tc<DP, NS, tc::kModeKfp0T>(b, status, st)          \
   : mode == tc::kModeBnd ? launch_tc<DP, NS, tc::kModeBnd>(b, status, st)            \
                          : launch_tc<DP, NS, tc::kModeFp0T>(b, status, st))
  if (a.d <= 8) return PDEIP_TC_DISPATCH(8, 2);
  if (a.d <= 16) return PDEIP_TC_DISPATCH(16, 1);
  return PDEIP_TC_DISPATCH(32, 1);
#undef PDEIP_TC_DISPATCH
}
#endif

int tensor_path_status(cudaStream_t st, int* out) {
  int* status = tensor_status_word();
  if (!status) return PDEIP_ERR_CUDA;
  int w[2] = {0, 0};
  if (cudaMemcpyAsync(w, status, 2 * sizeof(int), cudaMemcpyDeviceToHost, st) != cudaSuccess) return PDEIP_ERR_CUDA;
  if (cudaStreamSynchronize(st) != cudaSuccess) return PDEIP_ERR_CUDA;
  *out = (w[0] ? 1 : 0) | (w[1] ? 2 : 0);
  if (*out && cudaMemsetAsync(status, 0, 2 * sizeof(int), st) != cudaSuccess) return PDEIP_ERR_CUDA;
  return PDEIP_OK;
}

}

extern "C" int pdeip_tensor_path_status(void* stream, int* out_status) {
  PDEIP_REQUIRE(out_status != nullptr, PDEIP_ERR_INVALID_ARG, "out_status is NULL");
  return pdeip::tensor_path_status((cudaStream_t)stream, out_status);
}

extern "C" int pdeip_debug_set_status(int word, int value, void* stream) {
  int* status = pdeip::tensor_status_word();
  if (!status || word < 0 || word > 1) return PDEIP_ERR_INVALID_ARG;
  if (cudaMemcpyAsync(status + word, &value, sizeof(int), cudaMemcpyHostToDevice, (cudaStream_t)stream) != cudaSuccess)
    return PDEIP_ERR_CUDA;
  if (cudaStreamSynchronize((cudaStream_t)stream) != cudaSuccess) return PDEIP_ERR_CUDA;
  return PDEIP_OK;
}

extern "C" int pdeip_debug_tensor_trace(long long* out, int n) {
  int* status = pdeip::tensor_status_word();
  if (!status) return PDEIP_ERR_CUDA;
  if (n > 24 * 8 + 48 + 16) return PDEIP_ERR_INVALID_ARG;
  if (cudaDeviceSynchronize() != cudaSuccess) return PDEIP_ERR_CUDA;
  if (cudaMemcpy(out, reinterpret_cast<long long*>(status) + 512, sizeof(long long) * (size_t)n, cudaMemcpyDeviceToHost) !=
      cudaSuccess)
    return PDEIP_ERR_CUDA;
  if (cudaMemset(reinterpret_cast<long long*>(status) + 512, 0, sizeof(long long) * (size_t)n) != cudaSuccess)
    return PDEIP_ERR_CUDA;
  return PDEIP_OK;
}

extern "C" int pdeip_debug_tensor_probe(float* out, int n_floats) {
  int* status = pdeip::tensor_status_word();
  if (!status) return PDEIP_ERR_CUDA;
  if (n_floats > 24 * 128 * 48) return PDEIP_ERR_INVALID_ARG;
  if (cudaDeviceSynchronize() != cudaSuccess) return PDEIP_ERR_CUDA;
  if (cudaMemcpy(out, reinterpret_cast<float*>(status) + 2048, sizeof(float) * (size_t)n_floats, cudaMemcpyDeviceToHost) !=
      cudaSuccess)
    return PDEIP_ERR_CUDA;
  return PDEIP_OK;
}
```

Before: 2.195 billion.

## Widen tensor-path epilogue to 16 warps, spilling bias-grad accumulators to TMEM

For the single-stage configuration, the epilogue team doubles from 8 to 16 warps, so each warp handles a quarter of the hidden columns instead of half. Per-thread register budgets are lowered to match, and an OutCols helper splits output columns across parts. Running bias-gradient accumulators move into spare TMEM columns and scalar loss sums move to shared memory, which frees registers. Input loads are split so the drift band is fetched in a later phase. The aim is more latency hiding from extra warps, at the cost of more TMEM traffic and tighter register budgets that could spill.

After: 2.396 billion, median of 6. +9.2%, better.

```diff
diff --git a/pde_inverse_problem_b200/csrc/residual_tensor.cu b/pde_inverse_problem_b200/csrc/residual_tensor.cu
--- a/pde_inverse_problem_b200/csrc/residual_tensor.cu
+++ b/pde_inverse_problem_b200/csrc/residual_tensor.cu
@@ -29,10 +29,21 @@
 
 constexpr uint32_t C_AOP = C_SLOT0 + SLOT_COLS;
 constexpr uint32_t C_AOPX = C_AOP + 48;
+constexpr uint32_t C_DB = C_AOPX + 48;
+static_assert(C_DB + 4 * 26 == 512, "TMEM column map");
 
 constexpr int ZC_ZA2 = 0, ZC_ZA1 = 6, ZC_ZA0 = 10, ZC_TA = 14, ZC_TB = 20;
 constexpr int AC_T = 0, AC_A1 = 4, AC_C = 8;
 
+template <int NS>
+struct Team {
+  static constexpr int kEpiWarps = NS == 1 ? 16 : 8;
+  static constexpr int kParts = kEpiWarps / 4;
+  static constexpr int kEpiThreads = 32 * kEpiWarps;
+  static constexpr int kThreads = kEpiThreads + 32;
+  static constexpr int kLaunchThreads = kEpiThreads + 128;
+  static constexpr int kLaunchRegs = 65536 / kLaunchThreads / 8 * 8;
+};
 template <int DP, int NS>
 struct Cfg {
   static constexpr int XC = DP / 8;
@@ -64,8 +75,9 @@
 #define PDEIP_TC_STAGE 0
 #endif
   static constexpr uint32_t STAGE_BYTES = (PDEIP_TC_STAGE && NS == 1) ? 128u * 3u * DP * 4u : 0u;
+  static constexpr uint32_t SUMS_BYTES = NS == 1 ? 5u * 4u * Team<NS>::kEpiThreads : 0u;
   static constexpr uint32_t O_TRUE = O_BIAS + 512, O_MISC = O_TRUE + TP_BYTES, O_STAGE = O_MISC + 128,
-                            TOTAL = O_STAGE + STAGE_BYTES;
+                            O_SUMS = O_STAGE + STAGE_BYTES, TOTAL = O_SUMS + SUMS_BYTES;
   static_assert(TOTAL <= 227u * 1024u && O_STAGE % 128 == 0 && O_X2 % 1024 == 0, "shared-memory budget");
 };
 
@@ -81,11 +93,8 @@
 #ifndef PDEIP_TC_LO_FWD
 #define PDEIP_TC_LO_FWD true
 #endif
-constexpr int kEpiThreads = 256;
-constexpr int kThreads = kEpiThreads + 32;
-constexpr int kLaunchThreads = 384;
 #ifndef PDEIP_TC_REGS1_EPI
-#define PDEIP_TC_REGS1_EPI 232
+#define PDEIP_TC_REGS1_EPI 104
 #define PDEIP_TC_REGS1_MMA 40
 #endif
 #ifndef PDEIP_TC_REGS2_EPI
@@ -96,7 +105,9 @@
 struct Regs {
   static constexpr int kEpi = NS == 2 ? PDEIP_TC_REGS2_EPI : PDEIP_TC_REGS1_EPI;
   static constexpr int kMma = NS == 2 ? PDEIP_TC_REGS2_MMA : PDEIP_TC_REGS1_MMA;
-  static_assert(2 * (kEpi - 168) <= 168 - kMma && kEpi % 8 == 0 && kMma % 8 == 0 && kMma >= 24 && kEpi <= 256,
+  static constexpr int kEpiPerSched = Team<NS>::kEpiWarps / 4, kLaunch = Team<NS>::kLaunchRegs;
+  static_assert(kEpiPerSched * kEpi + kMma <= (kEpiPerSched + 1) * kLaunch && kEpi >= kLaunch && kMma <= kLaunch &&
+                    kEpi % 8 == 0 && kMma % 8 == 0 && kMma >= 24 && kEpi <= 256,
                 "setmaxnreg budgets: an impossible request never returns (the kernel hangs)");
 };
 
@@ -128,15 +139,21 @@
 #else
 #define TC_PROBE(id, unit0, arr, n) do { } while (0)
 #endif
-
-template <bool PROXY_FENCE = true>
+#define TC_PROBE_OUT(id, arr)                                                                       \
+  do {                                                                                              \
+    TC_PROBE(id, oc.unit0(), arr, 8 * OutCols<NP>::NC);                                             \
+    if constexpr (OutCols<NP>::PAIR) TC_PROBE(id, oc.pair_unit(), (arr) + 8 * OutCols<NP>::NC, 2); \
+  } while (0)
+
+template <int NS, bool PROXY_FENCE = true>
 __device__ __forceinline__ void epi_arrive(int slot) {
   if constexpr (PROXY_FENCE) fence_async_smem();
   fence_before_sync();
-  asm volatile("bar.arrive %0, %1;" ::"r"(1 + slot), "n"(kThreads) : "memory");
-}
+  asm volatile("bar.arrive %0, %1;" ::"r"(1 + slot), "n"(Team<NS>::kThreads) : "memory");
+}
+template <int NS>
 __device__ __forceinline__ void mma_wait_operands(int slot) {
-  asm volatile("bar.sync %0, %1;" ::"r"(1 + slot), "n"(kThreads) : "memory");
+  asm volatile("bar.sync %0, %1;" ::"r"(1 + slot), "n"(Team<NS>::kThreads) : "memory");
   fence_after_sync();
 }
 
@@ -326,19 +343,39 @@
                "r"(r[2]), "r"(r[3])
                : "memory");
 }
+__device__ __forceinline__ void tm_ld2(uint32_t taddr, uint32_t* r) {
+  asm volatile("tcgen05.ld.sync.aligned.32x32b.x2.b32 {%0,%1}, [%2];" : "=r"(r[0]), "=r"(r[1]) : "r"(taddr) : "memory");
+}
+__device__ __forceinline__ void tm_ld1(uint32_t taddr, uint32_t* r) {
+  asm volatile("tcgen05.ld.sync.aligned.32x32b.x1.b32 {%0}, [%1];" : "=r"(r[0]) : "r"(taddr) : "memory");
+}
+__device__ __forceinline__ void tm_st2(uint32_t taddr, const uint32_t* r) {
+  asm volatile("tcgen05.st.sync.aligned.32x32b.x2.b32 [%0], {%1,%2};" ::"r"(taddr), "r"(r[0]), "r"(r[1]) : "memory");
+}
+__device__ __forceinline__ void tm_st1(uint32_t taddr, uint32_t r) {
+  asm volatile("tcgen05.st.sync.aligned.32x32b.x1.b32 [%0], {%1};" ::"r"(taddr), "r"(r) : "memory");
+}
 template <int NU>
 __device__ __forceinline__ void tm_ldf(uint32_t taddr, float* v) {
   uint32_t* r = reinterpret_cast<uint32_t*>(v);
-  tm_ld16(taddr, r);
-  if constexpr (NU == 24) tm_ld8(taddr + 16, r + 16);
+  if constexpr (NU == 8) {
+    tm_ld8(taddr, r);
+  } else {
+    tm_ld16(taddr, r);
+    if constexpr (NU == 24) tm_ld8(taddr + 16, r + 16);
+  }
 }
 template <int NU>
 __device__ __forceinline__ void tm_ldp(uint32_t taddr, uint32_t* r) {
-  tm_ld8(taddr, r);
-  if constexpr (NU == 24) tm_ld4(taddr + 8, r + 8);
+  if constexpr (NU == 8) {
+    tm_ld4(taddr, r);
+  } else {
+    tm_ld8(taddr, r);
+    if constexpr (NU == 24) tm_ld4(taddr + 8, r + 8);
+  }
 }
 template <int NU>
-__device__ __forceinline__ void tm_park(uint32_t taddr, const float* v) {
+__device__ __forceinline__ void tm_park_st(uint32_t taddr, const float* v) {
   uint32_t r[NU / 2];
 #pragma unroll
   for (int i = 0; i < NU / 2; ++i) r[i] = pack2(v[2 * i], v[2 * i + 1]);
@@ -348,8 +385,53 @@
     tm_st8(taddr, r);
     if constexpr (NU == 24) tm_st4(taddr + 8, r + 8);
   }
+}
+template <int NU>
+__device__ __forceinline__ void tm_park(uint32_t taddr, const float* v) {
+  tm_park_st<NU>(taddr, v);
   tm_wait_st();
 }
+
+template <int NP>
+struct OutCols {
+  static constexpr int NC = NP == 2 ? 3 : 1;
+  static constexpr bool PAIR = NP == 4;
+  static constexpr int NU = 8 * NC + (PAIR ? 2 : 0);
+  const int part;
+  __device__ __forceinline__ int unit0() const { return 8 * NC * part; }
+  __device__ __forceinline__ int chunk0() const { return NC * part; }
+  __device__ __forceinline__ int pair_unit() const { return 32 + 2 * part; }
+  __device__ __forceinline__ int unit(int i) const { return i < 8 * NC ? unit0() + i : pair_unit() + i - 8 * NC; }
+  __device__ __forceinline__ void ldf(uint32_t taddr, float* v) const {
+    tm_ldf<8 * NC>(taddr + unit0(), v);
+    if constexpr (PAIR) tm_ld2(taddr + pair_unit(), reinterpret_cast<uint32_t*>(v + 8 * NC));
+  }
+  __device__ __forceinline__ void ldp(uint32_t taddr, uint32_t* r) const {
+    tm_ldp<8 * NC>(taddr + 4 * NC * part, r);
+    if constexpr (PAIR) tm_ld1(taddr + 16 + part, r + 4 * NC);
+  }
+  __device__ __forceinline__ void park(uint32_t taddr, const float* v) const {
+    tm_park_st<8 * NC>(taddr + 4 * NC * part, v);
+    if constexpr (PAIR) tm_st1(taddr + 16 + part, pack2(v[8 * NC], v[8 * NC + 1]));
+    tm_wait_st();
+  }
+  __device__ __forceinline__ void ld_smem(const float* b, float* v) const {
+#pragma unroll
+    for (int i = 0; i < 2 * NC; ++i)
+      *reinterpret_cast<float4*>(v + 4 * i) = *reinterpret_cast<const float4*>(b + unit0() + 4 * i);
+    if constexpr (PAIR) *reinterpret_cast<float2*>(v + 8 * NC) = *reinterpret_cast<const float2*>(b + pair_unit());
+  }
+  template <bool TS>
+  __device__ __forceinline__ void put(uint8_t* row, int c0, uint32_t w0, const float* v) const {
+#pragma unroll
+    for (int c = 0; c < NC; ++c) put_op<TS>(row, (c0 + NC * part + c) * 128, w0 + 4 * (NC * part + c), v + 8 * c);
+    if constexpr (PAIR) {
+      const uint32_t w = pack2(v[8 * NC], v[8 * NC + 1]);
+      *reinterpret_cast<uint32_t*>(row + (c0 + 4) * 128 + 4 * part) = w;
+      if constexpr (TS) tm_st1(w0 + 16 + part, w);
+    }
+  }
+};
 
 template <int DP>
 __device__ __noinline__ void true_grad_chunk(const ResidualArgs& a, const float* __restrict__ tp, int64_t p, int dimw,
@@ -417,7 +499,7 @@
 
 constexpr int kModeKfp0T = 0, kModeBnd = 1, kModeFp0T = 2;
 template <int DP, int NS, int MODE>
-__global__ void __launch_bounds__(kLaunchThreads, 1) mlp_residual_tc_kernel(const ResidualArgs a, int* status) {
+__global__ void __launch_bounds__(Team<NS>::kLaunchThreads, 1) mlp_residual_tc_kernel(const ResidualArgs a, int* status) {
   constexpr bool BND = MODE == kModeBnd, FPM = MODE == kModeFp0T;
 #ifndef PDEIP_TC_TS
 #define PDEIP_TC_TS 1
@@ -434,11 +516,15 @@
   constexpr bool kPipeX = Cfg<DP, NS>::PIPE_X;
   constexpr bool kPipeFlow = kPipeX;
   using S = Cfg<DP, NS>;
+  constexpr int kEpiThreads = Team<NS>::kEpiThreads, kThreads = Team<NS>::kThreads, kLaunchThreads = Team<NS>::kLaunchThreads;
+  constexpr int NP = Team<NS>::kParts;
+  constexpr int UH = 32 / NP;
+  constexpr int HC = UH / 8;
   extern __shared__ __align__(1024) uint8_t sm[];
   const int tid = threadIdx.x, warp = tid >> 5, lane = tid & 31;
   const bool is_mma_warp = warp == kEpiThreads / 32;
   const int q = warp & 3;
-  const int half = (warp >> 2) & 1;
+  const int part = warp >> 2;
   const int row = q * 32 + lane;
   const int d = a.d;
   const MlpShape<H> sh{d, 2};
@@ -570,7 +656,7 @@
             }
           };
           TC_TRACE_DECL_MMA;
-          mma_wait_operands(s);
+          mma_wait_operands<NS>(s);
           if (elect_one()) {
             TC_TRACE(4);
             switch (ph) {
@@ -738,12 +824,32 @@
 #ifdef PDEIP_TC_PROBE
     float* probe = reinterpret_cast<float*>(status) + 2048;
 #endif
-    float db0[16], db1[16], db2[24];
-#pragma unroll
-    for (int i = 0; i < 16; ++i) { db0[i] = 0.f; db1[i] = 0.f; }
-#pragma unroll
-    for (int i = 0; i < 24; ++i) db2[i] = 0.f;
+    const OutCols<NP> oc{part};
+    constexpr int UO = OutCols<NP>::NU;
+    constexpr bool kDbTmem = NS == 1;
+    static_assert(!kDbTmem || (UH == 8 && UO == 10), "C_DB map: 8 + 8 + 10 columns per part");
+    const uint32_t LDB = TB + ((uint32_t)(q * 32) << 16) + C_DB;
+    const uint32_t cdb0 = LDB + 8 * part, cdb1 = LDB + 32 + 8 * part, cdb2 = LDB + 64 + 8 * part, cdb2p = LDB + 96 + 2 * part;
+    auto db_ld = [&](uint32_t col, float* v) { tm_ld8(col, reinterpret_cast<uint32_t*>(v)); };
+    auto db_st = [&](uint32_t col, const float* v) { tm_st8(col, reinterpret_cast<const uint32_t*>(v)); };
+    auto db2_ld = [&](float* v) { db_ld(cdb2, v); tm_ld2(cdb2p, reinterpret_cast<uint32_t*>(v + 8)); };
+    auto db2_st = [&](const float* v) { db_st(cdb2, v); tm_st2(cdb2p, reinterpret_cast<const uint32_t*>(v + 8)); };
+    float db0[UH], db1[UH], db2[UO];
+#pragma unroll
+    for (int i = 0; i < UH; ++i) { db0[i] = 0.f; db1[i] = 0.f; }
+#pragma unroll
+    for (int i = 0; i < UO; ++i) db2[i] = 0.f;
+    if constexpr (kDbTmem) {
+      db_st(cdb0, db0);
+      db_st(cdb1, db1);
+      db2_st(db2);
+      tm_wait_st();
+    }
+    constexpr bool kSumsSmem = NS == 1;
+    float* const sums_s = reinterpret_cast<float*>(sm + S::O_SUMS) + tid;
     float sum_g2 = 0.f, sum_gt2 = 0.f, sum_gd2 = 0.f, sum_d1 = 0.f, sum_d2 = 0.f;
+    if constexpr (kSumsSmem)
+      for (int k = 0; k < 5; ++k) sums_s[k * kEpiThreads] = 0.f;
     const float gamma = a.coef, gamma4 = 4.f * a.coef;
     const float cgw = 1.f / (float)fpd;
     const int dimw = (FPM ? d : 2 * d) + (a.tg.kind == PDEIP_DRIFT_IN_POINTS ? d : 0);
@@ -752,23 +858,23 @@
     const uint32_t offZ = (uint32_t)(row & 7) * 16u + (uint32_t)(row >> 3) * S::RG_Z;
     const uint32_t LA0 = TB + ((uint32_t)(q * 32) << 16) + C_SLOT0;
     const uint32_t LOP = TB + ((uint32_t)(q * 32) << 16) + C_AOP;
-    const int u16 = 16 * half, u24 = 24 * half;
-    constexpr int NI = (3 * S::XC + 1) / 2;
+    const int uh = UH * part;
+    constexpr int NI = (3 * S::XC + NP - 1) / NP;
     float xin0[NI][8], xin1[NI][8];
     const bool fast_in = !FPM && a.layout == PDEIP_LAYOUT_BLOCK128 && d == DP;
-    auto load_into = [&](float (&xin)[NI][8], int64_t t, const int i0 = 0, const int i1 = 64) {
+    auto load_into = [&](float (&xin)[NI][8], int64_t t, const int bands = 7) {
       if (fast_in) {
         const int64_t pp = t * 128 + row;
         const bool inside = t < n_tiles && pp < a.n_points;
-        const float* const pb = a.points + (inside ? t * (int64_t)(128 * dimw) + row : (int64_t)0) + half * (8 * 128);
+        const float* const pb = a.points + (inside ? t * (int64_t)(128 * dimw) + row : (int64_t)0) + part * (8 * 128);
         const bool has_gt = a.tg.kind == PDEIP_DRIFT_IN_POINTS;
 #pragma unroll
         for (int i = 0; i < NI; ++i) {
-          if (i < i0 || i >= i1) continue;
-          if (half + 2 * i >= 3 * S::XC) continue;
-          if (half + 2 * i >= 2 * S::XC && !has_gt) continue;
-#pragma unroll
-          for (int e = 0; e < 8; ++e) xin[i][e] = __ldg(pb + (16 * i + e) * 128);
+          if (part + NP * i >= 3 * S::XC) continue;
+          if (!((bands >> ((part + NP * i) / S::XC)) & 1)) continue;
+          if (part + NP * i >= 2 * S::XC && !has_gt) continue;
+#pragma unroll
+          for (int e = 0; e < 8; ++e) xin[i][e] = __ldg(pb + (8 * NP * i + e) * 128);
         }
         return;
       }
@@ -780,8 +886,8 @@
       const float* const pbase = a.points + point_base(a.layout, pc, dimw);
 #pragma unroll
       for (int i = 0; i < NI; ++i) {
-        if (i < i0 || i >= i1) continue;
-        const int j = half + 2 * i;
+        const int j = part + NP * i;
+        if (j < 3 * S::XC && !((bands >> (j / S::XC)) & 1)) continue;
         const int band = (j / S::XC) < 3 ? (j / S::XC) : 0, cg = j % S::XC;
         const int bandc = (band < 2 || a.tg.kind == PDEIP_DRIFT_IN_POINTS) ? band : 0;
         const int bandm = FPM ? (bandc == 2 ? 1 : 0) : bandc;
@@ -807,9 +913,9 @@
       bulk_g2s(smem_u32(sm + S::O_STAGE), a.points + pt * 128 * dimw, bytes, stage_mbar);
     };
     if (use_stage && tid == 0) stage_issue(tile_begin);
-    auto load_inputs = [&](int s, int64_t t, const int i0 = 0, const int i1 = 64) {
-      if (NS == 2 && s == 1) load_into(xin1, t, i0, i1);
-      else load_into(xin0, t, i0, i1);
+    auto load_inputs = [&](int s, int64_t t, const int bands = 7) {
+      if (NS == 2 && s == 1) load_into(xin1, t, bands);
+      else load_into(xin0, t, bands);
     };
 #ifndef PDEIP_TC_L2_PREFETCH
 #define PDEIP_TC_L2_PREFETCH 1
@@ -817,11 +923,11 @@
     auto prefetch_inputs = [&](int64_t t) {
       if (FPM || t >= n_tiles || (t + 1) * 128 > a.n_points) return;
       if (a.layout == PDEIP_LAYOUT_SOA) {
-        if ((a.n_points & 3) == 0 && half == 0 && row < dimw)
+        if ((a.n_points & 3) == 0 && part == 0 && row < dimw)
           asm volatile("cp.async.bulk.prefetch.L2.global [%0], %1;" ::"l"(a.points + (int64_t)row * a.n_points + t * 128),
                        "r"(512u)
                        : "memory");
-      } else if (half == 0 && row == 0) {
+      } else if (part == 0 && row == 0) {
         asm volatile("cp.async.bulk.prefetch.L2.global [%0], %1;" ::"l"(a.points + t * 128 * dimw),
                      "r"((uint32_t)(512 * dimw))
                      : "memory");
@@ -840,7 +946,7 @@
     auto emit_x = [&](const float (&xin)[NI][8], const bool valid_t, uint8_t* const Xd) {
 #pragma unroll
       for (int i = 0; i < NI; ++i) {
-        const int j = half + 2 * i;
+        const int j = part + NP * i;
         const int band = j / S::XC, cg = j % S::XC;
         if (band == 0) {
           float hi[8], lo[8];
@@ -896,7 +1002,10 @@
       constexpr bool kEarlyLoads = true;
 #if PDEIP_TC_L2_PREFETCH
       if constexpr (ph == 0) {
-        if (!use_stage) load_inputs(s, tile);
+        if (!use_stage) load_inputs(s, tile, kPipeFlow ? 3 : 7);
+      }
+      if constexpr (kPipeFlow && ph == 5) {
+        if (a.tg.kind == PDEIP_DRIFT_IN_POINTS) load_inputs(s, tile, 4);
       }
 #endif
       if constexpr (kStage && ph == 0) {
@@ -909,7 +1018,7 @@
           const int dir = FPM ? (int)((uint32_t)tile % fpd) : -1;
 #pragma unroll
           for (int i = 0; i < NI; ++i) {
-            const int j = half + 2 * i;
+            const int j = part + NP * i;
             const int band = (j / S::XC) < 3 ? (j / S::XC) : 0, cg = j % S::XC;
             if (band < 2) {
 #pragma unroll
@@ -929,19 +1038,19 @@
       } else if constexpr (ph == 1 || ph == 2) {
         constexpr bool l1 = ph == 1;
         uint8_t* const At = l1 ? A1 : A2;
-        float z0[16], z1[16], z2[16];
-        tm_ldf<16>(LA + (l1 ? C_Z0 : C_Z1) + u16, z0);
-        tm_ldf<16>(LA + (l1 ? C_Z10 : C_Z11) + u16, z1);
-        if constexpr (!l1) tm_ldf<16>(LA + C_Z21 + u16, z2);
-        float bb[16];
-#pragma unroll
-        for (int i = 0; i < 4; ++i)
-          *reinterpret_cast<float4*>(bb + 4 * i) = *reinterpret_cast<const float4*>(bias_s + (l1 ? 0 : 32) + u16 + 4 * i);
+        float z0[UH], z1[UH], z2[UH];
+        tm_ldf<UH>(LA + (l1 ? C_Z0 : C_Z1) + uh, z0);
+        tm_ldf<UH>(LA + (l1 ? C_Z10 : C_Z11) + uh, z1);
+        if constexpr (!l1) tm_ldf<UH>(LA + C_Z21 + uh, z2);
+        float bb[UH];
+#pragma unroll
+        for (int i = 0; i < UH / 4; ++i)
+          *reinterpret_cast<float4*>(bb + 4 * i) = *reinterpret_cast<const float4*>(bias_s + (l1 ? 0 : 32) + uh + 4 * i);
         tm_wait_ld();
-        float t[16], s1[16], q1[16], q2[16];
+        float t[UH], s1[UH], q1[UH], q2[UH];
 #if PDEIP_TC_PACKED
 #pragma unroll
-        for (int i = 0; i < 8; ++i) {
+        for (int i = 0; i < UH / 2; ++i) {
           const float2 zb = __fadd2_rn(pr(z0, i), pr(bb, i));
           const float2 t2 = make_float2(tanh_fast(zb.x), tanh_fast(zb.y));
           const float2 s2 = __ffma2_rn(__fmul2_rn(t2, bc2(-1.f)), t2, bc2(1.f));
@@ -953,7 +1062,7 @@
         }
 #else
 #pragma unroll
-        for (int i = 0; i < 16; ++i) {
+        for (int i = 0; i < UH; ++i) {
           t[i] = tanh_fast(z0[i] + bb[i]);
           s1[i] = fmaf(-t[i], t[i], 1.f);
           q1[i] = s1[i] * z1[i];
@@ -962,34 +1071,32 @@
         }
 #endif
 #pragma unroll
-        for (int c = 0; c < 2; ++c) {
-          put_op<kTS>(At, (AC_T + 2 * half + c) * 128, LOP + 4 * (AC_T + 2 * half + c), t + 8 * c);
-          put_op<kTS>(At, (AC_A1 + 2 * half + c) * 128, LOP + 4 * (AC_A1 + 2 * half + c), q1 + 8 * c);
-          put_op<kTS>(At, (AC_C + 2 * half + c) * 128, LOP + 4 * (AC_C + 2 * half + c), q2 + 8 * c);
-        }
-        tm_park<16>(LA + (l1 ? C_S1P1 : C_S1P2) + 8 * half, s1);
-        TC_PROBE(l1 ? 0 : 3, u16, t, 16);
-        TC_PROBE(l1 ? 1 : 4, u16, q1, 16);
-        TC_PROBE(l1 ? 2 : 5, u16, q2, 16);
+        for (int c = 0; c < HC; ++c) {
+          put_op<kTS>(At, (AC_T + HC * part + c) * 128, LOP + 4 * (AC_T + HC * part + c), t + 8 * c);
+          put_op<kTS>(At, (AC_A1 + HC * part + c) * 128, LOP + 4 * (AC_A1 + HC * part + c), q1 + 8 * c);
+          put_op<kTS>(At, (AC_C + HC * part + c) * 128, LOP + 4 * (AC_C + HC * part + c), q2 + 8 * c);
+        }
+        tm_park<UH>(LA + (l1 ? C_S1P1 : C_S1P2) + UH / 2 * part, s1);
+        TC_PROBE(l1 ? 0 : 3, uh, t, UH);
+        TC_PROBE(l1 ? 1 : 4, uh, q1, UH);
+        TC_PROBE(l1 ? 2 : 5, uh, q2, UH);
       } else if constexpr (ph == 3) {
-        float u[24], u1[24], u2[24];
-        tm_ldf<24>(LA + C_U + u24, u);
-        tm_ldf<24>(LA + C_U1 + u24, u1);
-        tm_ldf<24>(LA + C_U2 + u24, u2);
-        float bb[24];
-#pragma unroll
-        for (int i = 0; i < 6; ++i)
-          *reinterpret_cast<float4*>(bb + 4 * i) = *reinterpret_cast<const float4*>(bias_s + 64 + u24 + 4 * i);
+        float u[UO], u1[UO], u2[UO];
+        oc.ldf(LA + C_U, u);
+        oc.ldf(LA + C_U1, u1);
+        oc.ldf(LA + C_U2, u2);
+        float bb[UO];
+        oc.ld_smem(bias_s + 64, bb);
         tm_wait_ld();
         const float k8 = BND ? 0.f : 8.f * mk, kg = (BND ? 2.f * a.coef : gamma4) * mk;
         float d1 = 0.f, d2a = 0.f, d2b = 0.f;
-        float za[24], sv[24], sp[24];
+        float za[UO], sv[UO], sp[UO];
 #if PDEIP_TC_PACKED
         {
           float2 e1 = bc2(0.f), e2a = bc2(0.f), e2b = bc2(0.f);
           const float2 k82 = bc2(k8), nk82 = bc2(-k8), kg2 = bc2(kg);
 #pragma unroll
-          for (int i = 0; i < 12; ++i) {
+          for (int i = 0; i < UO / 2; ++i) {
             const float2 uu = __fadd2_rn(pr(u, i), pr(bb, i));
             const float2 v1 = pr(u1, i), v2 = pr(u2, i);
             e1 = __ffma2_rn(uu, v1, e1);
@@ -1003,7 +1110,7 @@
         }
 #else
 #pragma unroll
-        for (int i = 0; i < 24; ++i) {
+        for (int i = 0; i < UO; ++i) {
           const float uu = u[i] + bb[i];
           d1 = fmaf(uu, u1[i], d1);
           d2a = fmaf(u1[i], u1[i], d2a);
@@ -1013,39 +1120,44 @@
           sp[i] = fmaf(k8, u2[i], kg * u1[i]);
         }
 #endif
-#pragma unroll
-        for (int c = 0; c < 3; ++c) {
-          put_op<kTS>(Z, (ZC_ZA2 + 3 * half + c) * 128, LOP + 4 * (3 * half + c), za + 8 * c);
-          put_op<kTS>(Z, (ZC_TA + 3 * half + c) * 128, LOP + 24 + 4 * (3 * half + c), sv + 8 * c);
-        }
-        tm_park<24>(LA + C_S0P + 12 * half, sp);
+        oc.template put<kTS>(Z, ZC_ZA2, LOP, za);
+        oc.template put<kTS>(Z, ZC_TA, LOP + 24, sv);
+        oc.park(LA + C_S0P, sp);
+        if constexpr (kSumsSmem) {
+          sum_d1 = sums_s[3 * kEpiThreads];
+          sum_d2 = sums_s[4 * kEpiThreads];
+        }
         sum_d1 = fmaf(2.f * mk, d1, sum_d1);
         sum_d2 = fmaf(mk, 2.f * d2a - 4.f * d2b, sum_d2);
-        TC_PROBE(6, u24, za, 24);
-        TC_PROBE(7, u24, sv, 24);
-        TC_PROBE(8, u24, sp, 24);
+        if constexpr (kSumsSmem) {
+          sums_s[3 * kEpiThreads] = sum_d1;
+          sums_s[4 * kEpiThreads] = sum_d2;
+        }
+        TC_PROBE_OUT(6, za);
+        TC_PROBE_OUT(7, sv);
+        TC_PROBE_OUT(8, sp);
       } else if constexpr (ph == 4 || ph == 5) {
         if constexpr (kPipeFlow && ph == 4) prefetch_inputs(tile + tile_stride);
         constexpr bool l2 = ph == 4;
         const uint8_t* At = l2 ? A2 : A1;
-        float aa[16], ab1[16], t[16], a1[16];
-        uint32_t s1p[8];
-        tm_ldp<16>(LA + (l2 ? C_S1P2 : C_S1P1) + 8 * half, s1p);
-#pragma unroll
-        for (int c = 0; c < 2; ++c) {
-          load_chunk(At, (AC_T + 2 * half + c) * 128, t + 8 * c);
-          load_chunk(At, (AC_A1 + 2 * half + c) * 128, a1 + 8 * c);
+        float aa[UH], ab1[UH], t[UH], a1[UH];
+        uint32_t s1p[UH / 2];
+        tm_ldp<UH>(LA + (l2 ? C_S1P2 : C_S1P1) + UH / 2 * part, s1p);
+#pragma unroll
+        for (int c = 0; c < HC; ++c) {
+          load_chunk(At, (AC_T + HC * part + c) * 128, t + 8 * c);
+          load_chunk(At, (AC_A1 + HC * part + c) * 128, a1 + 8 * c);
         }
         tm_wait_ld();
         if constexpr (kEarlyLoads) wait_gemm();
-        tm_ldf<16>(LA + (l2 ? C_AA2 : C_AA1) + u16, aa);
-        tm_ldf<16>(LA + (l2 ? C_AB12 : C_AB11) + u16, ab1);
+        tm_ldf<UH>(LA + (l2 ? C_AA2 : C_AA1) + uh, aa);
+        tm_ldf<UH>(LA + (l2 ? C_AB12 : C_AB11) + uh, ab1);
         tm_wait_ld();
         TC_FINE(0);
-        float za[16], zb[16], pz[16];
+        float za[UH], zb[UH], pz[UH];
 #if PDEIP_TC_PACKED
 #pragma unroll
-        for (int i = 0; i < 8; ++i) {
+        for (int i = 0; i < UH / 2; ++i) {
           const float2 s2 = unp2(s1p, i), aa2 = pr(aa, i), a12 = pr(a1, i), ab2 = pr(ab1, i);
           const float2 tt = __fmul2_rn(pr(t, i), bc2(2.f));
           const float2 qq = __fmul2_rn(aa2, a12);
@@ -1055,7 +1167,7 @@
         }
 #else
 #pragma unroll
-        for (int i = 0; i < 16; ++i) {
+        for (int i = 0; i < UH; ++i) {
           const float s1 = unp(s1p, i);
           za[i] = aa[i] * s1;
           const float qq = aa[i] * a1[i];
@@ -1064,129 +1176,160 @@
         }
 #endif
 #pragma unroll
-        for (int c = 0; c < 2; ++c) {
-          put_op<kTS>(Z, ((l2 ? ZC_ZA1 : ZC_ZA0) + 2 * half + c) * 128, LOP + 4 * (2 * half + c), za + 8 * c);
-          put_op<(kTS && l2)>(Z, ((l2 ? ZC_TB : ZC_TA) + 2 * half + c) * 128, LOP + 16 + 4 * (2 * half + c), zb + 8 * c);
+        for (int c = 0; c < HC; ++c) {
+          put_op<kTS>(Z, ((l2 ? ZC_ZA1 : ZC_ZA0) + HC * part + c) * 128, LOP + 4 * (HC * part + c), za + 8 * c);
+          put_op<(kTS && l2)>(Z, ((l2 ? ZC_TB : ZC_TA) + HC * part + c) * 128, LOP + 16 + 4 * (HC * part + c), zb + 8 * c);
         }
         TC_FINE(1);
-        tm_park<16>(LA + (l2 ? C_PZ2 : C_PZ1) + 8 * half, pz);
+        tm_park<UH>(LA + (l2 ? C_PZ2 : C_PZ1) + UH / 2 * part, pz);
         TC_FINE(2);
-        TC_PROBE(l2 ? 9 : 12, u16, za, 16);
-        TC_PROBE(l2 ? 10 : 13, u16, zb, 16);
-        TC_PROBE(l2 ? 11 : 14, u16, pz, 16);
+        TC_PROBE(l2 ? 9 : 12, uh, za, UH);
+        TC_PROBE(l2 ? 10 : 13, uh, zb, UH);
+        TC_PROBE(l2 ? 11 : 14, uh, pz, UH);
       } else if constexpr (ph == 6) {
+        if constexpr (kSumsSmem) {
+          sum_g2 = sums_s[0];
+          sum_gt2 = sums_s[kEpiThreads];
+          sum_gd2 = sums_s[2 * kEpiThreads];
+        }
+        const bool gt_stored = a.tg.kind == PDEIP_DRIFT_IN_POINTS;
+        const float mkc = mk * cgw;
+        auto add_sums = [&](const float* gv, const float* gt) {
+#pragma unroll
+          for (int e = 0; e < 8; ++e) {
+            const float df = gt[e] - gv[e];
+            sum_g2 = fmaf(mkc * gv[e], gv[e], sum_g2);
+            sum_gt2 = fmaf(mkc * gt[e], gt[e], sum_gt2);
+            sum_gd2 = fmaf(mkc * df, df, sum_gd2);
+          }
+        };
+        auto g_chunk = [&](int cg, float* gv) {
+          tm_ld8(LA + C_G + 8 * cg, reinterpret_cast<uint32_t*>(gv));
+          tm_wait_ld();
+#pragma unroll
+          for (int e = 0; e < 8; ++e) gv[e] *= 0.25f;
+        };
 #pragma unroll
         for (int i = 0; i < NI; ++i) {
-          const int j = half + 2 * i;
+          const int j = part + NP * i;
           const int band = j / S::XC, cg = j % S::XC;
-          const bool own_sum = a.tg.kind == PDEIP_DRIFT_IN_POINTS ? band == 2 : band == 0;
-          if (j < 3 * S::XC && (band == 0 || own_sum)) {
-            float g4[8], gv[8], gt[8];
-            tm_ld8(LA + C_G + 8 * cg, reinterpret_cast<uint32_t*>(g4));
-            tm_wait_ld();
-#pragma unroll
-            for (int e = 0; e < 8; ++e) {
-              gv[e] = 0.25f * g4[e];
-              gt[e] = 0.f;
-            }
-            if (band == 0) {
-              float gh[8];
-#pragma unroll
-              for (int e = 0; e < 8; ++e) gh[e] = (0.125f * cgw) * g4[e];
-              put_op<kTS>(X, (S::XC_G + cg) * 128, LOP + 4 * cg, gh);
-              TC_PROBE(15, cg * 8, gv, 8);
-            }
-            if (own_sum) {
-              const float mkc = mk * cgw;
-              if (a.tg.kind == PDEIP_DRIFT_IN_POINTS) {
-#pragma unroll
-                for (int e = 0; e < 8; ++e) {
-                  const int u = cg * 8 + e;
-                  float val;
-                  if (kStage && use_stage) val = stage[((FPM ? d : 2 * d) + (u < d ? u : 0)) * 128];
-                  else val = (NS == 2 && s == 1) ? xin1[i][e] : xin0[i][e];
-                  gt[e] = (valid && u < d) ? val : 0.f;
-                }
-              } else if (a.tg.kind == PDEIP_DRIFT_LINEAR || a.tg.kind == PDEIP_DRIFT_GMM) {
-                true_grad_chunk<DP>(a, tp, valid ? p : (int64_t)-1, dimw, cg, gt);
+          if (band == 0) {
+            float gv[8], gh[8];
+            g_chunk(cg, gv);
+#pragma unroll
+            for (int e = 0; e < 8; ++e) gh[e] = (0.5f * cgw) * gv[e];
+            put_op<kTS>(X, (S::XC_G + cg) * 128, LOP + 4 * cg, gh);
+            TC_PROBE(15, cg * 8, gv, 8);
+          }
+        }
+        if (gt_stored) {
+#pragma unroll
+          for (int i = 0; i < NI; ++i) {
+            const int j = part + NP * i;
+            const int band = j / S::XC, cg = j % S::XC;
+            if (j < 3 * S::XC && band == 2) {
+              float gv[8], gt[8];
+              g_chunk(cg, gv);
+#pragma unroll
+              for (int e = 0; e < 8; ++e) {
+                const int u = cg * 8 + e;
+                float val;
+                if (kStage && use_stage) val = stage[((FPM ? d : 2 * d) + (u < d ? u : 0)) * 128];
+                else val = (NS == 2 && s == 1) ? xin1[i][e] : xin0[i][e];
+                gt[e] = (valid && u < d) ? val : 0.f;
               }
-#pragma unroll
-              for (int e = 0; e < 8; ++e) {
-                const float df = gt[e] - gv[e];
-                sum_g2 = fmaf(mkc * gv[e], gv[e], sum_g2);
-                sum_gt2 = fmaf(mkc * gt[e], gt[e], sum_gt2);
-                sum_gd2 = fmaf(mkc * df, df, sum_gd2);
-              }
+              add_sums(gv, gt);
             }
           }
+        } else {
+#pragma unroll
+          for (int i = 0; i < NI; ++i) {
+            const int j = part + NP * i;
+            const int band = j / S::XC, cg = j % S::XC;
+            if (band == 0) {
+              float gv[8], gt[8];
+              g_chunk(cg, gv);
+#pragma unroll
+              for (int e = 0; e < 8; ++e) gt[e] = 0.f;
+              if (a.tg.kind == PDEIP_DRIFT_LINEAR || a.tg.kind == PDEIP_DRIFT_GMM)
+                true_grad_chunk<DP>(a, tp, valid ? p : (int64_t)-1, dimw, cg, gt);
+              add_sums(gv, gt);
+            }
+          }
+        }
+        if constexpr (kSumsSmem) {
+          sums_s[0] = sum_g2;
+          sums_s[kEpiThreads] = sum_gt2;
+          sums_s[2 * kEpiThreads] = sum_gd2;
         }
       } else if constexpr (ph == 7 || ph == 8) {
         constexpr bool l1 = ph == 7;
         uint8_t* const At = l1 ? A1 : A2;
-        float zg[16], a2[16];
-        uint32_t s1p[8];
-        tm_ldp<16>(LA + (l1 ? C_S1P1 : C_S1P2) + 8 * half, s1p);
-#pragma unroll
-        for (int c = 0; c < 2; ++c) load_chunk(At, (AC_C + 2 * half + c) * 128, a2 + 8 * c);
+        float zg[UH], a2[UH];
+        uint32_t s1p[UH / 2];
+        tm_ldp<UH>(LA + (l1 ? C_S1P1 : C_S1P2) + UH / 2 * part, s1p);
+#pragma unroll
+        for (int c = 0; c < HC; ++c) load_chunk(At, (AC_C + HC * part + c) * 128, a2 + 8 * c);
         tm_wait_ld();
         if constexpr (kEarlyLoads && !(kGram && l1)) wait_gemm();
         if constexpr (kStage && l1) {
           if (use_stage && tid == 0) stage_issue(tile + tile_stride);
         }
-        tm_ldf<16>(LA + (l1 ? C_ZG0 : C_ZG1) + u16, zg);
+        tm_ldf<UH>(LA + (l1 ? C_ZG0 : C_ZG1) + uh, zg);
         tm_wait_ld();
-        float ag[16], cc[16];
+        float ag[UH], cc[UH];
 #if PDEIP_TC_PACKED
 #pragma unroll
-        for (int i = 0; i < 8; ++i) {
+        for (int i = 0; i < UH / 2; ++i) {
           const float2 g2 = __fmul2_rn(unp2(s1p, i), pr(zg, i));
           st2(ag, i, g2);
           st2(cc, i, __fadd2_rn(pr(a2, i), g2));
         }
 #else
 #pragma unroll
-        for (int i = 0; i < 16; ++i) {
+        for (int i = 0; i < UH; ++i) {
           ag[i] = unp(s1p, i) * zg[i];
           cc[i] = a2[i] + ag[i];
         }
 #endif
 #pragma unroll
-        for (int c = 0; c < 2; ++c) {
-          put_op<kTS>(At, (AC_A1 + 2 * half + c) * 128, LOP + 4 * (2 * half + c), ag + 8 * c);
-          put_chunk(At, (AC_C + 2 * half + c) * 128, cc + 8 * c);
-        }
-        TC_PROBE(l1 ? 16 : 17, u16, cc, 16);
+        for (int c = 0; c < HC; ++c) {
+          put_op<kTS>(At, (AC_A1 + HC * part + c) * 128, LOP + 4 * (HC * part + c), ag + 8 * c);
+          put_chunk(At, (AC_C + HC * part + c) * 128, cc + 8 * c);
+        }
+        TC_PROBE(l1 ? 16 : 17, uh, cc, UH);
       } else if constexpr (ph == 9) {
-        float ug[24], s0[24];
-        uint32_t spp[12];
-        tm_ldp<24>(LA + C_S0P + 12 * half, spp);
+        float ug[UO], s0[UO];
+        uint32_t spp[UO / 2];
+        oc.ldp(LA + C_S0P, spp);
+        if constexpr (kDbTmem) db2_ld(db2);
         tm_wait_ld();
         if constexpr (kEarlyLoads) wait_gemm();
-        tm_ldf<24>(LA + C_UG + u24, ug);
+        oc.ldf(LA + C_UG, ug);
         tm_wait_ld();
 #if PDEIP_TC_PACKED
 #pragma unroll
-        for (int i = 0; i < 12; ++i) {
+        for (int i = 0; i < UO / 2; ++i) {
           const float2 v = __ffma2_rn(bc2(8.f), pr(ug, i), unp2(spp, i));
           st2(s0, i, v);
           st2(db2, i, __fadd2_rn(pr(db2, i), v));
         }
 #else
 #pragma unroll
-        for (int i = 0; i < 24; ++i) {
+        for (int i = 0; i < UO; ++i) {
           s0[i] = fmaf(8.f, ug[i], unp(spp, i));
           db2[i] += s0[i];
         }
 #endif
-#pragma unroll
-        for (int c = 0; c < 3; ++c) put_op<kTS>(Z, (ZC_TA + 3 * half + c) * 128, LOP + 4 * (3 * half + c), s0 + 8 * c);
-        TC_PROBE(18, u24, s0, 24);
+        oc.template put<kTS>(Z, ZC_TA, LOP, s0);
+        if constexpr (kDbTmem) db2_st(db2);
+        TC_PROBE_OUT(18, s0);
       } else {
         constexpr bool l2 = ph == 10;
 #if PDEIP_TC_L2_PREFETCH
         if constexpr (l2) {
           if constexpr (kPipeFlow) {
-            if (tile + tile_stride < n_tiles) load_inputs(s, tile + tile_stride, 0, 2);
+            if (tile + tile_stride < n_tiles) load_inputs(s, tile + tile_stride, 3);
           } else if (!use_stage) {
             prefetch_inputs(tile + tile_stride);
           }
@@ -1195,24 +1338,25 @@
         if constexpr (l2) load_inputs(s, tile + tile_stride);
 #endif
         const uint8_t* At = l2 ? A2 : A1;
-        float ab[16], aa[16], t[16], cc[16];
-        uint32_t s1p[8], pzp[8];
-        tm_ldp<16>(LA + (l2 ? C_S1P2 : C_S1P1) + 8 * half, s1p);
-        tm_ldp<16>(LA + (l2 ? C_PZ2 : C_PZ1) + 8 * half, pzp);
-#pragma unroll
-        for (int c = 0; c < 2; ++c) {
-          load_chunk(At, (AC_T + 2 * half + c) * 128, t + 8 * c);
-          load_chunk(At, (AC_C + 2 * half + c) * 128, cc + 8 * c);
-        }
+        float ab[UH], aa[UH], t[UH], cc[UH];
+        uint32_t s1p[UH / 2], pzp[UH / 2];
+        tm_ldp<UH>(LA + (l2 ? C_S1P2 : C_S1P1) + UH / 2 * part, s1p);
+        tm_ldp<UH>(LA + (l2 ? C_PZ2 : C_PZ1) + UH / 2 * part, pzp);
+#pragma unroll
+        for (int c = 0; c < HC; ++c) {
+          load_chunk(At, (AC_T + HC * part + c) * 128, t + 8 * c);
+          load_chunk(At, (AC_C + HC * part + c) * 128, cc + 8 * c);
+        }
+        if constexpr (kDbTmem) db_ld(l2 ? cdb1 : cdb0, l2 ? db1 : db0);
         tm_wait_ld();
         if constexpr (kEarlyLoads) wait_gemm();
-        tm_ldf<16>(LA + (l2 ? C_AB2 : C_AB1) + u16, ab);
-        tm_ldf<16>(LA + (l2 ? C_AA2R : C_AA1R) + u16, aa);
+        tm_ldf<UH>(LA + (l2 ? C_AB2 : C_AB1) + uh, ab);
+        tm_ldf<UH>(LA + (l2 ? C_AA2R : C_AA1R) + uh, aa);
         tm_wait_ld();
-        float zb[16];
+        float zb[UH];
 #if PDEIP_TC_PACKED
 #pragma unroll
-        for (int i = 0; i < 8; ++i) {
+        for (int i = 0; i < UH / 2; ++i) {
           const float2 m0 = __ffma2_rn(unp2(s1p, i), pr(ab, i), unp2(pzp, i));
           const float2 ta = __fmul2_rn(__fmul2_rn(pr(t, i), bc2(-2.f)), pr(aa, i));
           const float2 v = __ffma2_rn(ta, pr(cc, i), m0);
@@ -1222,7 +1366,7 @@
         }
 #else
 #pragma unroll
-        for (int i = 0; i < 16; ++i) {
+        for (int i = 0; i < UH; ++i) {
           const float m0 = fmaf(unp(s1p, i), ab[i], unp(pzp, i));
           zb[i] = fmaf(-2.f * t[i] * aa[i], cc[i], m0);
           if (l2) db1[i] += zb[i];
@@ -1230,15 +1374,16 @@
         }
 #endif
 #pragma unroll
-        for (int c = 0; c < 2; ++c)
-          put_op<(kTS && l2)>(Z, ((l2 ? ZC_TB : ZC_TA) + 2 * half + c) * 128, LOP + 4 * (2 * half + c), zb + 8 * c);
-        TC_PROBE(l2 ? 19 : 20, u16, zb, 16);
+        for (int c = 0; c < HC; ++c)
+          put_op<(kTS && l2)>(Z, ((l2 ? ZC_TB : ZC_TA) + HC * part + c) * 128, LOP + 4 * (HC * part + c), zb + 8 * c);
+        if constexpr (kDbTmem) db_st(l2 ? cdb1 : cdb0, l2 ? db1 : db0);
+        TC_PROBE(l2 ? 19 : 20, uh, zb, UH);
       }
       if constexpr (!(kGram && ph == 6)) {
         if constexpr (kTS) tm_wait_st();
         TC_TRACE(7);
         if constexpr (kTwoStage && (ph == 3 || ph == 4 || ph == 5 || ph == 7 || ph == 9 || ph == 10 || ph == 11)) {
-          epi_arrive<false>(s);
+          epi_arrive<NS, false>(s);
           fence_async_smem();
           asm volatile("bar.arrive %0, %1;" ::"r"(4 + (int)tsb), "n"(kThreads) : "memory");
           tsb ^= 1u;
@@ -1251,7 +1396,7 @@
         asm volatile("bar.arrive %0, %1;" ::"r"(1 + s), "n"(kThreads) : "memory");
 #else
         constexpr bool kNeedProxyFence = !(kTS && (ph == 0 || ph == 1 || ph == 2 || ph == 8));
-        epi_arrive<kNeedProxyFence>(s);
+        epi_arrive<NS, kNeedProxyFence>(s);
 #endif
         }
         TC_TRACE(2);
@@ -1259,10 +1404,7 @@
       if constexpr (kPipeFlow && ph == 10) {
         const int64_t tn = tile + tile_stride;
         const int64_t pn = (FPM ? (int64_t)((uint32_t)tn / fpd) : tn) * 128 + row;
-        if (tn < n_tiles) {
-          load_inputs(s, tn, 2, 64);
-          emit_x(xin0, pn < a.n_points, sm + (xb ? 0u : S::O_X2) + S::O_X + offX);
-        }
+        if (tn < n_tiles) emit_x(xin0, pn < a.n_points, sm + (xb ? 0u : S::O_X2) + S::O_X + offX);
       }
     };
 #define PDEIP_TC_PHASE(PH)                       \
@@ -1287,43 +1429,57 @@
     fence_after_sync();
     asm volatile("bar.sync 3, %0;" ::"n"(kEpiThreads) : "memory");
 
-    float* part = a.ws + (int64_t)blockIdx.x * a.pstride;
+    float* wsp = a.ws + (int64_t)blockIdx.x * a.pstride;
     float* red = reinterpret_cast<float*>(sm);
+    static_assert((512 + 8 * Team<NS>::kEpiWarps) * 4 <= S::O_BIAS, "write-out scratch inside the operand tiles");
     const float wt = a.weight;
     if (ok && q < 2) {
       const uint32_t LQ = TB + ((uint32_t)(q * 32) << 16);
       const int iu = 16 * q + lane;
-      float w2[24], w1[16], w0[16];
-      tm_ldf<24>(LQ + C_DW2 + u24, w2);
-      tm_ldf<16>(LQ + C_DW1 + u16, w1);
-      tm_ldf<16>(LQ + C_DW0 + u16, w0);
+      float w2[UO], w1[UH], w0[UH];
+      oc.ldf(LQ + C_DW2, w2);
+      tm_ldf<UH>(LQ + C_DW1 + uh, w1);
+      tm_ldf<UH>(LQ + C_DW0 + uh, w0);
       tm_wait_ld();
       if (lane < 16) {
 #pragma unroll
-        for (int i = 0; i < 24; ++i)
-          if (u24 + i < kOut) part[sh.w_off(2) + iu * kOut + u24 + i] += wt * w2[i];
-#pragma unroll
-        for (int i = 0; i < 16; ++i) part[sh.w_off(1) + iu * H + u16 + i] += wt * w1[i];
+        for (int i = 0; i < UO; ++i)
+          if (oc.unit(i) < kOut) wsp[sh.w_off(2) + iu * kOut + oc.unit(i)] += wt * w2[i];
+#pragma unroll
+        for (int i = 0; i < UH; ++i) wsp[sh.w_off(1) + iu * H + uh + i] += wt * w1[i];
         if (iu < d) {
 #pragma unroll
-          for (int i = 0; i < 16; ++i) part[sh.w_off(0) + iu * H + u16 + i] += wt * w0[i];
-        }
-      }
-    }
-#pragma unroll
-    for (int i = 0; i < 16; ++i) {
+          for (int i = 0; i < UH; ++i) wsp[sh.w_off(0) + iu * H + uh + i] += wt * w0[i];
+        }
+      }
+    }
+    if constexpr (kDbTmem) {
+      db_ld(cdb0, db0);
+      db_ld(cdb1, db1);
+      db2_ld(db2);
+      tm_wait_ld();
+    }
+#pragma unroll
+    for (int i = 0; i < UH; ++i) {
       const float r0 = warp_sum(db0[i]), r1 = warp_sum(db1[i]);
       if (lane == 0) {
-        red[q * 128 + u16 + i] = r0;
-        red[q * 128 + 32 + u16 + i] = r1;
-      }
-    }
-#pragma unroll
-    for (int i = 0; i < 24; ++i) {
+        red[q * 128 + uh + i] = r0;
+        red[q * 128 + 32 + uh + i] = r1;
+      }
+    }
+#pragma unroll
+    for (int i = 0; i < UO; ++i) {
       const float r2 = warp_sum(db2[i]);
-      if (lane == 0) red[q * 128 + 64 + u24 + i] = r2;
+      if (lane == 0) red[q * 128 + 64 + oc.unit(i)] = r2;
     }
     {
+      if constexpr (kSumsSmem) {
+        sum_g2 = sums_s[0];
+        sum_gt2 = sums_s[kEpiThreads];
+        sum_gd2 = sums_s[2 * kEpiThreads];
+        sum_d1 = sums_s[3 * kEpiThreads];
+        sum_d2 = sums_s[4 * kEpiThreads];
+      }
       const float sums5[5] = {sum_g2, sum_gt2, sum_gd2, sum_d1, sum_d2};
 #pragma unroll
       for (int k = 0; k < 5; ++k) {
@@ -1335,25 +1491,25 @@
     if (ok) {
       if (tid < 112) {
         const float v = (red[tid] + red[128 + tid]) + (red[256 + tid] + red[384 + tid]);
-        if (tid < 32) part[sh.b_off(0) + tid] += wt * v;
-        else if (tid < 64) part[sh.b_off(1) + tid - 32] += wt * v;
-        else if (tid - 64 < kOut) part[sh.b_off(2) + tid - 64] += wt * v;
+        if (tid < 32) wsp[sh.b_off(0) + tid] += wt * v;
+        else if (tid < 64) wsp[sh.b_off(1) + tid - 32] += wt * v;
+        else if (tid - 64 < kOut) wsp[sh.b_off(2) + tid - 64] += wt * v;
       }
       if (tid == 128) {
         float t5[5] = {0.f, 0.f, 0.f, 0.f, 0.f};
-        for (int w = 0; w < kEpiThreads / 32; ++w)
+        for (int w = 0; w < Team<NS>::kEpiWarps; ++w)
           for (int k = 0; k < 5; ++k) t5[k] += red[512 + w * 8 + k];
         const float g2 = wt * t5[0], gt2 = wt * t5[1], gd2 = wt * t5[2], D1 = wt * t5[3], D2 = wt * t5[4];
         if constexpr (BND) {
-          part[P + PDEIP_SUM_BOUNDARY] += a.coef * D1;
-          part[P + PDEIP_SUM_LOSS] += a.coef * D1;
+          wsp[P + PDEIP_SUM_BOUNDARY] += a.coef * D1;
+          wsp[P + PDEIP_SUM_LOSS] += a.coef * D1;
         } else {
-          part[P + PDEIP_SUM_G2] += g2;
-          part[P + PDEIP_SUM_GTRUE2] += gt2;
-          part[P + PDEIP_SUM_GT] += gd2;
-          if (!FPM) part[P + PDEIP_SUM_D1] += D1;
-          part[P + PDEIP_SUM_D2] += D2;
-          part[P + PDEIP_SUM_LOSS] += g2 + gt2 - 2.f * D2 + 2.f * gamma * D1;
+          wsp[P + PDEIP_SUM_G2] += g2;
+          wsp[P + PDEIP_SUM_GTRUE2] += gt2;
+          wsp[P + PDEIP_SUM_GT] += gd2;
+          if (!FPM) wsp[P + PDEIP_SUM_D1] += D1;
+          wsp[P + PDEIP_SUM_D2] += D2;
+          wsp[P + PDEIP_SUM_LOSS] += g2 + gt2 - 2.f * D2 + 2.f * gamma * D1;
         }
       }
     }
@@ -1385,7 +1541,7 @@
   PDEIP_REQUIRE(true_grad_floats(a.tg, a.d) * sizeof(float) <= S::TP_BYTES, PDEIP_ERR_UNSUPPORTED,
                 "tensor path: true-gradient parameters exceed %u bytes", (unsigned)S::TP_BYTES);
   PDEIP_CUDA_OK(cudaFuncSetAttribute(kern, cudaFuncAttributeMaxDynamicSharedMemorySize, (int)S::TOTAL));
-  kern<<<residual_grid(), tc::kLaunchThreads, S::TOTAL, st>>>(a, status);
+  kern<<<residual_grid(), tc::Team<NS>::kLaunchThreads, S::TOTAL, st>>>(a, status);
   PDEIP_LAUNCH_OK();
   return PDEIP_OK;
 }
```
